# floe/backscrub

Hardware: AMD Instinct MI355X
Metric: composited frames/sec at 640×480 (batch), 1/2/4/8 MI355X + mask IoU vs CPU ref (higher is better)
Workload: dtype f32 (network) / u8 (image kernels)

## Files before the change

backscrub_amd/api.py:

```python
from __future__ import annotations

import ctypes as C
import os

import numpy as np

_HERE = os.path.dirname(os.path.abspath(__file__))
_LIB = None

_u8p = C.POINTER(C.c_uint8)
DEBUG_FN = C.CFUNCTYPE(None, C.c_void_p, C.c_char_p)
STAGE_FN = C.CFUNCTYPE(None, C.c_void_p)


class BsxError(RuntimeError):
    pass


class _Info(C.Structure):
    _fields_ = [("model_type", C.c_int), ("width", C.c_int), ("height", C.c_int), ("n_streams", C.c_int),
                ("in_w", C.c_int), ("in_h", C.c_int), ("in_c", C.c_int), ("out_w", C.c_int), ("out_h", C.c_int),
                ("out_c", C.c_int), ("roi", C.c_int * 4), ("in_roi", C.c_int * 4), ("n_ops", C.c_int), ("n_steps", C.c_int),
                ("device", C.c_int), ("norm_scale", C.c_float), ("norm_offset", C.c_float), ("nn_flops_per_frame", C.c_double),
                ("act_bytes_per_stream", C.c_size_t)]


class LaunchStat(C.Structure):
    _fields_ = [("name", C.c_char * 64), ("avg_ms", C.c_double), ("bytes", C.c_double), ("flops", C.c_double)]


SYMBOLS = [
    ("bsx_version", C.c_char_p, []),
    ("bsx_device_count", C.c_int, []),
    ("bsx_new", C.c_void_p, [C.c_char_p, C.c_size_t, C.c_size_t, C.c_size_t, C.c_int, C.c_int, DEBUG_FN, STAGE_FN, STAGE_FN, STAGE_FN, C.c_void_p]),
    ("bsx_delete", None, [C.c_void_p]),
    ("bsx_get_info", C.c_int, [C.c_void_p, C.POINTER(_Info)]),
    ("bsx_last_error", C.c_char_p, [C.c_void_p]),
    ("bsx_reset", C.c_int, [C.c_void_p, C.c_void_p]),
    ("bsx_process_host", C.c_int, [C.c_void_p, C.c_int, C.c_void_p, C.c_size_t, C.c_void_p, C.c_size_t]),
    ("bsx_process_batch", C.c_int, [C.c_void_p, C.c_void_p, C.c_int, C.c_void_p, C.c_void_p]),
    ("bsx_masks_device", C.c_void_p, [C.c_void_p]),
    ("bsx_composite_batch", C.c_int, [C.c_void_p, C.c_void_p, C.c_size_t, C.c_void_p, C.c_void_p, C.c_void_p, C.c_int, C.c_void_p]),
    ("bsx_step_batch", C.c_int, [C.c_void_p, C.c_void_p, C.c_void_p, C.c_size_t, C.c_void_p, C.c_int, C.c_void_p]),
    ("bsx_step_batch_yuyv", C.c_int, [C.c_void_p, C.c_void_p, C.c_void_p, C.c_size_t, C.c_void_p, C.c_int, C.c_void_p]),
    ("bsx_step_batch_ex", C.c_int, [C.c_void_p, C.c_void_p, C.c_void_p, C.c_size_t, C.c_void_p, C.c_int, C.c_void_p, C.c_uint]),
    ("bsx_step_batch_pipelined", C.c_int, [C.c_void_p, C.c_void_p, C.c_void_p, C.c_size_t, C.c_void_p, C.c_int, C.c_void_p, C.c_uint]),
    ("bsx_step_batch_vcam", C.c_int, [C.c_void_p, C.c_void_p, C.c_void_p, C.c_size_t, C.c_void_p, C.c_int, C.c_int, C.c_int, C.c_void_p, C.c_uint]),
    ("bsx_resize_bgr", C.c_int, [C.c_void_p, C.c_void_p, C.c_int, C.c_int, C.c_void_p, C.c_int, C.c_int, C.c_int, C.c_void_p]),
    ("bsx_bgr_to_yuyv", C.c_int, [C.c_void_p, C.c_void_p, C.c_void_p, C.c_int, C.c_int, C.c_int, C.c_void_p]),
    ("bsx_yuyv_to_bgr", C.c_int, [C.c_void_p, C.c_void_p, C.c_void_p, C.c_int, C.c_int, C.c_int, C.c_void_p]),
    ("bsx_background_load", C.c_void_p, [C.c_void_p, C.c_char_p, C.c_int]),
    ("bsx_background_from_frames", C.c_void_p, [C.c_void_p, C.c_void_p, C.c_int, C.c_int, C.c_int, C.c_double, C.c_int]),
    ("bsx_background_free", None, [C.c_void_p]),
    ("bsx_background_info", C.c_int, [C.c_void_p, C.POINTER(C.c_int), C.POINTER(C.c_int), C.POINTER(C.c_int), C.POINTER(C.c_double), C.POINTER(C.c_int)]),
    ("bsx_background_grab", C.c_int, [C.c_void_p, C.c_int, C.c_int, C.c_void_p, C.c_void_p]),
    ("bsx_media_decode", C.c_int, [C.c_char_p, C.POINTER(C.c_int), C.POINTER(C.c_int), C.POINTER(C.c_double), C.POINTER(C.POINTER(C.c_uint8)), C.c_char_p, C.c_size_t]),
    ("bsx_media_free", None, [C.POINTER(C.c_uint8)]),
    ("bsx_live_new", C.c_void_p, [C.c_void_p]),
    ("bsx_live_delete", None, [C.c_void_p]),
    ("bsx_live_set_input_frame", C.c_int, [C.c_void_p, C.c_void_p, C.c_size_t]),
    ("bsx_live_get_output_mask", C.c_int, [C.c_void_p, C.c_void_p, C.c_size_t]),
    ("bsx_live_timings", C.c_int, [C.c_void_p, C.POINTER(C.c_long), C.POINTER(C.c_long)]),
    ("bsx_gaussian_blur_bgr", C.c_int, [C.c_void_p, C.c_void_p, C.c_void_p, C.c_int, C.c_int, C.c_int, C.c_int, C.c_void_p]),
    ("bsx_debug_gauss_coeffs", C.c_int, [C.c_int, C.c_int, C.POINTER(C.c_uint32), C.POINTER(C.c_uint32)]),
    ("bsx_flip_bgr", C.c_int, [C.c_void_p, C.c_void_p, C.c_void_p, C.c_int, C.c_int, C.c_int, C.c_int, C.c_void_p]),
    ("bsx_debug_buffer", C.c_int, [C.c_void_p, C.c_int, C.POINTER(C.c_void_p), C.POINTER(C.c_size_t)]),
    ("bsx_debug_run_stage", C.c_int, [C.c_void_p, C.c_int, C.c_void_p, C.c_int, C.c_void_p]),
    ("bsx_plan_describe", C.c_char_p, [C.c_void_p]),
    ("bsx_debug_tensor", C.c_long, [C.c_void_p, C.c_int, C.POINTER(C.c_float), C.c_long]),
    ("bsx_model_precompile", C.c_int, [C.c_char_p, C.c_char_p, C.c_char_p, C.c_size_t]),
    ("bsx_model_kernel_source", C.c_long, [C.c_char_p, C.c_char_p, C.c_size_t]),
    ("bsx_model_seg_source", C.c_long, [C.c_char_p, C.c_char_p, C.c_size_t]),
    ("bsx_debug_tensor_of", C.c_long, [C.c_void_p, C.c_int, C.c_int, C.POINTER(C.c_float), C.c_long]),
    ("bsx_debug_mask_tile_stats", C.c_int, [C.c_void_p, C.c_int, C.POINTER(C.c_long)]),
    ("bsx_debug_program_timeline", C.c_int, [C.c_void_p, C.c_int, C.POINTER(C.c_ulonglong), C.c_int, C.c_void_p]),
    ("bsx_model_describe", C.c_int, [C.c_char_p, C.c_char_p, C.c_size_t]),
    ("bsx_profile_batch", C.c_int, [C.c_void_p, C.c_void_p, C.c_void_p, C.c_size_t, C.c_void_p, C.c_int, C.c_int, C.POINTER(LaunchStat), C.c_int, C.c_void_p]),
]


def lib_path() -> str:
    return os.environ.get("BSX_LIBRARY") or os.path.join(_HERE, "libbsx.so")


def lib():
    global _LIB
    if _LIB is None:
        import torch
        p = lib_path()
        if not os.path.exists(p):
            raise BsxError("libbsx.so is missing (%s): run `python -m backscrub_amd.build` — there is no CPU fallback" % p)
        L = C.CDLL(p)
        for name, res, args in SYMBOLS:
            f = getattr(L, name)
            f.restype = res
            f.argtypes = args
        _LIB = L
    return _LIB


def _check(rc, ctx=None, what=""):
    if rc != 0:
        msg = lib().bsx_last_error(ctx) or b""
        raise BsxError("%s failed (%d): %s" % (what, rc, msg.decode(errors="replace").strip()))


def _torch():
    import torch
    return torch


def _stream_ptr():
    torch = _torch()
    return C.c_void_p(torch.cuda.current_stream().cuda_stream)


class MaskGen:

    def __init__(self, model_path, width, height, n_streams=1, device=0, threads=2, ondebug=None, onprep=None, oninfer=None,
                 onmask=None, caller_ctx=None):
        L = lib()
        self._cbs = (DEBUG_FN(ondebug) if ondebug else DEBUG_FN(), STAGE_FN(onprep) if onprep else STAGE_FN(),
                     STAGE_FN(oninfer) if oninfer else STAGE_FN(), STAGE_FN(onmask) if onmask else STAGE_FN())
        self.h = L.bsx_new(os.fsencode(model_path), threads, width, height, n_streams, device, *self._cbs, caller_ctx)
        if not self.h:
            raise BsxError("bsx_new failed: %s" % (L.bsx_last_error(None) or b"").decode(errors="replace").strip())
        info = _Info()
        _check(L.bsx_get_info(self.h, C.byref(info)), self.h, "bsx_get_info")
        self.info = {k: (list(getattr(info, k)) if k in ("roi", "in_roi") else getattr(info, k)) for k, _ in _Info._fields_}
        self.width, self.height, self.n_streams, self.device = width, height, n_streams, device

    def process_batch(self, frames, masks_out=None):
        n = self._n(frames)
        mo = C.c_void_p(masks_out.data_ptr()) if masks_out is not None else None
        _check(lib().bsx_process_batch(self.h, C.c_void_p(frames.data_ptr()), n, mo, _stream_ptr()), self.h, "bsx_process_batch")
        return self.masks()[:n]

    def composite(self, bg, frames, masks=None, out=None):
        torch = _torch()
        n = self._n(frames)
        if out is None:
            out = torch.empty_like(frames)
        stride = self._bg(bg, n)
        mp = C.c_void_p(masks.data_ptr()) if masks is not None else None
        _check(lib().bsx_composite_batch(self.h, C.c_void_p(bg.data_ptr()), stride, C.c_void_p(frames.data_ptr()), mp,
                                         C.c_void_p(out.data_ptr()), n, _stream_ptr()), self.h, "bsx_composite_batch")
        return out

    def _bg(self, bg, n):
        ok = (bg.dtype == _torch().uint8 and bg.is_cuda and bg.dim() in (3, 4) and tuple(bg.shape[-3:]) == (self.height, self.width, 3)
              and tuple(bg.stride()[-3:]) == (self.width * 3, 3, 1) and (bg.dim() == 3 or bg.shape[0] >= n) and bg.device.index == self.device
              and (bg.dim() == 3 or bg.stride(0) >= 0))
        if not ok:
            raise BsxError("bg must be a cuda:%d uint8 tensor [%d,%d,3] or [>=%d,%d,%d,3] with contiguous images" % (self.device, self.height, self.width, n, self.height, self.width))
        return 0 if bg.dim() == 3 else int(bg.stride(0))

    def step(self, frames, bg, out):
# ... 95 lines not shown
        self._release_pending()

    def resize_bgr(self, src, dw, dh):
        torch = _torch()
        n, sh, sw, _ = src.shape
        dst = torch.empty((n, dh, dw, 3), dtype=torch.uint8, device=src.device)
        _check(lib().bsx_resize_bgr(self.h, C.c_void_p(src.data_ptr()), sw, sh, C.c_void_p(dst.data_ptr()), dw, dh, n, _stream_ptr()),
               self.h, "bsx_resize_bgr")
        return dst

    def bgr_to_yuyv(self, bgr):
        torch = _torch()
        n, h, w, _ = bgr.shape
        out = torch.empty((n, h, w, 2), dtype=torch.uint8, device=bgr.device)
        _check(lib().bsx_bgr_to_yuyv(self.h, C.c_void_p(bgr.data_ptr()), C.c_void_p(out.data_ptr()), w, h, n, _stream_ptr()),
               self.h, "bsx_bgr_to_yuyv")
        return out

    def flip_bgr(self, bgr, code):
        torch = _torch()
        n, h, w, _ = bgr.shape
        out = torch.empty_like(bgr)
        _check(lib().bsx_flip_bgr(self.h, C.c_void_p(bgr.data_ptr()), C.c_void_p(out.data_ptr()), w, h, n, int(code), _stream_ptr()), self.h, "bsx_flip_bgr")
        return out

    def gaussian_blur(self, bgr, ksize=25, out=None):
        torch = _torch()
        n, h, w, _ = bgr.shape
        if out is None:
            out = torch.empty_like(bgr)
        elif out.shape != bgr.shape or out.dtype != bgr.dtype or not out.is_contiguous() or out.device != bgr.device:
            raise BsxError("out must be a contiguous tensor shaped like the input")
        _check(lib().bsx_gaussian_blur_bgr(self.h, C.c_void_p(bgr.data_ptr()), C.c_void_p(out.data_ptr()), w, h, n, int(ksize), _stream_ptr()),
               self.h, "bsx_gaussian_blur_bgr")
        return out

    def yuyv_to_bgr(self, yuyv):
        torch = _torch()
        n, h, w, _ = yuyv.shape
        out = torch.empty((n, h, w, 3), dtype=torch.uint8, device=yuyv.device)
        _check(lib().bsx_yuyv_to_bgr(self.h, C.c_void_p(yuyv.data_ptr()), C.c_void_p(out.data_ptr()), w, h, n, _stream_ptr()),
               self.h, "bsx_yuyv_to_bgr")
        return out

    def process_host(self, frame: np.ndarray, stream_idx=0, mask_out: np.ndarray | None = None) -> np.ndarray:
        if frame.dtype != np.uint8 or frame.ndim != 3 or frame.shape[2] != 3 or frame.shape[0] != self.height or frame.shape[1] != self.width:
            raise BsxError("frame must be uint8 [%d,%d,3]" % (self.height, self.width))
        if frame.strides[2] != 1 or frame.strides[1] != 3:
            frame = np.ascontiguousarray(frame)
        if mask_out is None:
            mask_out = np.empty((self.height, self.width), np.uint8)
        elif (not isinstance(mask_out, np.ndarray) or mask_out.dtype != np.uint8 or mask_out.shape != (self.height, self.width)
              or mask_out.strides[1] != 1 or mask_out.strides[0] < self.width or not mask_out.flags.writeable):
            raise BsxError("mask_out must be a writable uint8 [%d,%d] array with unit inner stride" % (self.height, self.width))
        _check(lib().bsx_process_host(self.h, stream_idx, frame.ctypes.data, frame.strides[0], mask_out.ctypes.data, mask_out.strides[0]),
               self.h, "bsx_process_host")
        return mask_out

    def run_stage(self, stage, frames=None, n=None):
        n = n if n is not None else (self._n(frames, yuyv_in=(stage == 4)) if frames is not None else self.n_streams)
        fp = C.c_void_p(frames.data_ptr()) if frames is not None else None
        _check(lib().bsx_debug_run_stage(self.h, stage, fp, n, _stream_ptr()), self.h, "bsx_debug_run_stage")

    def input_tensor(self):
        i = self.info
        return self._view(0, "float32", (self.n_streams, i["in_h"], i["in_w"], i["in_c"]))

    def output_tensor(self):
        i = self.info
        return self._view(1, "float32", (self.n_streams, i["out_h"], i["out_w"], i["out_c"]))

    def ofinal(self):
        i = self.info
        return self._view(2, "uint8", (self.n_streams, i["out_h"], i["out_w"]))

    def plan(self) -> str:
        return lib().bsx_plan_describe(self.h).decode()

    def mask_tile_stats(self, n=None) -> dict:
        a = (C.c_long * 4)()
        _check(lib().bsx_debug_mask_tile_stats(self.h, n or self.n_streams, a), self.h, "bsx_debug_mask_tile_stats")
        return {"tiles": a[0], "uniform_255": a[1], "uniform_0": a[2], "general": a[3], "tile": "128x32"}

    def graph_tensor(self, idx, stream=None) -> np.ndarray:
        if stream is not None:
            n = lib().bsx_debug_tensor_of(self.h, idx, stream, None, 0)
            if n < 0:
                raise BsxError("tensor %d not materialised" % idx)
            a = np.empty(n, np.float32)
            lib().bsx_debug_tensor_of(self.h, idx, stream, a.ctypes.data_as(C.POINTER(C.c_float)), n)
            return a
        n = lib().bsx_debug_tensor(self.h, idx, None, 0)
        if n < 0:
            raise BsxError("tensor %d not materialised" % idx)
        _torch().cuda.synchronize()
        a = np.empty(n, np.float32)
        lib().bsx_debug_tensor(self.h, idx, a.ctypes.data_as(C.POINTER(C.c_float)), n)
        return a

    def _view(self, which, dtype, shape):
        torch = _torch()
        p, b = C.c_void_p(), C.c_size_t()
        _check(lib().bsx_debug_buffer(self.h, which, C.byref(p), C.byref(b)), self.h, "bsx_debug_buffer")
        return _as_torch(p.value, b.value, dtype, shape, self.device)

    def _n(self, frames, yuyv_in=False):
        ch = 2 if yuyv_in else 3
        if frames.dim() != 4 or tuple(frames.shape[1:]) != (self.height, self.width, ch) or not frames.is_contiguous() or not frames.is_cuda or frames.dtype != _torch().uint8:
            raise BsxError("frames must be a contiguous cuda uint8 tensor [n,%d,%d,%d]" % (self.height, self.width, ch))
        if frames.shape[0] > self.n_streams:
            raise BsxError("batch larger than n_streams")
        return int(frames.shape[0])

    def close(self):
        if getattr(self, "h", None):
            lib().bsx_delete(self.h)
            self.h = None

    def __del__(self):
        try:
            self.close()
        except Exception:
            pass


class _CudaArray:

    def __init__(self, ptr, nbytes, typestr, shape):
        self.__cuda_array_interface__ = {"shape": tuple(shape), "typestr": typestr, "data": (ptr, False), "version": 2, "strides": None}
        self._nbytes = nbytes


def _as_torch(ptr, nbytes, dtype, shape, device):
    torch = _torch()
    typestr = {"uint8": "|u1", "float32": "<f4"}[dtype]
    return torch.as_tensor(_CudaArray(ptr, nbytes, typestr, shape), device="cuda:%d" % device)


def media_decode(path: str):
    w, h, fps, ptr = C.c_int(), C.c_int(), C.c_double(), C.POINTER(C.c_uint8)()
    err = C.create_string_buffer(512)
    n = lib().bsx_media_decode(os.fsencode(path), C.byref(w), C.byref(h), C.byref(fps), C.byref(ptr), err, len(err))
    if n <= 0:
        raise BsxError(err.value.decode(errors="replace") or "media decode failed (%d)" % n)
    try:
        frames = np.ctypeslib.as_array(ptr, (n, h.value, w.value, 3)).copy()
    finally:
        lib().bsx_media_free(ptr)
    return frames, fps.value


class Background:

    def __init__(self, mg: MaskGen, path=None, frames=None, fps=0.0, debug=0):
        self.mg = mg
        if path is not None:
            self.h = lib().bsx_background_load(mg.h, os.fsencode(path), debug)
        else:
            frames = np.ascontiguousarray(frames, np.uint8)
            n, hh, ww, _ = frames.shape
            self.h = lib().bsx_background_from_frames(mg.h, frames.ctypes.data, ww, hh, n, float(fps), debug)
        if not self.h:
            raise BsxError("cannot load background")
        w, h, n, f, v = C.c_int(), C.c_int(), C.c_int(), C.c_double(), C.c_int()
        lib().bsx_background_info(self.h, C.byref(w), C.byref(h), C.byref(n), C.byref(f), C.byref(v))
        self.width, self.height, self.n_frames, self.fps, self.video = w.value, h.value, n.value, f.value, bool(v.value)
# ... 130 lines not shown
```

backscrub_amd/csrc/bsx_api.hip:

```cpp
#include "debug_switches.hpp"
#include <hip/hip_runtime.h>

#include <cmath>
#include <cstdarg>
#include <cstdio>
#include <cstdlib>
#include <cstring>
#include <map>
#include <memory>
#include <string>
#include <vector>

#include "../../include/bsx.h"
#include "gen_mid.hpp"
#include "gen_seg.hpp"
#include "kernels.hpp"
#include "roctx_ranges.hpp"
#include "rtc.hpp"
#include "plan.hpp"
#include "tflite_model.hpp"

using namespace bsx;

namespace {
thread_local std::string g_last_error;

struct HostResizeTab {
  std::vector<int> xofs, yofs;
  std::vector<short> xa, ya;
  int sw = 0, sh = 0, dw = 0, dh = 0, mode = 0;
};

inline int cv_floor(float v) { int i = (int)v; return i - (i > v); }
inline short sat_short(long v) { return (short)(v < -32768 ? -32768 : (v > 32767 ? 32767 : v)); }

HostResizeTab make_resize_tab(int sw, int sh, int dw, int dh) {
  HostResizeTab t;
  t.sw = sw; t.sh = sh; t.dw = dw; t.dh = dh;
  if (sw == dw && sh == dh) { t.mode = 1; return t; }
  double inv_x = (double)dw / sw, inv_y = (double)dh / sh;
  double scale_x = 1. / inv_x, scale_y = 1. / inv_y;
  long isx = lrint(scale_x), isy = lrint(scale_y);
  bool area_fast = std::fabs(scale_x - (double)isx) < 2.220446049250313e-16 && std::fabs(scale_y - (double)isy) < 2.220446049250313e-16;
  if (area_fast && isx == 2 && isy == 2) { t.mode = 2; return t; }
  t.xofs.resize(dw); t.xa.resize(2 * (size_t)dw); t.yofs.resize(dh); t.ya.resize(2 * (size_t)dh);
  for (int dx = 0; dx < dw; dx++) {
    float fx = (float)((dx + 0.5) * scale_x - 0.5);
    int sx = cv_floor(fx);
    fx -= sx;
    if (sx < 0) { fx = 0; sx = 0; }
    if (sx >= sw - 1) { fx = 0; sx = sw - 1; }
    t.xofs[dx] = sx;
    t.xa[2 * dx] = sat_short(lrintf((1.f - fx) * 2048.f));
    t.xa[2 * dx + 1] = sat_short(lrintf(fx * 2048.f));
  }
  for (int dy = 0; dy < dh; dy++) {
    float fy = (float)((dy + 0.5) * scale_y - 0.5);
    int sy = cv_floor(fy);
    fy -= sy;
    t.yofs[dy] = sy;
    t.ya[2 * dy] = sat_short(lrintf((1.f - fy) * 2048.f));
    t.ya[2 * dy + 1] = sat_short(lrintf(fy * 2048.f));
  }
  return t;
}

struct DevResizeTab {
  ResizeTab tab;
  void* mem = nullptr;
};
struct VcamTab {
  DevResizeTab d;
  bool direct = false;
};

}

struct bsx_ctx {
  bsx_debug_fn ondebug = nullptr;
  bsx_stage_fn onprep = nullptr, oninfer = nullptr, onmask = nullptr;
  void* caller_ctx = nullptr;
  Graph graph;
  Plan plan;
  int model_type = BSX_MODEL_UNKNOWN;
  float norm_scale = 0, norm_offset = 0;
  int width = 0, height = 0, n_streams = 0, device = 0;
  int inW = 0, inH = 0, inC = 0, outW = 0, outH = 0, outC = 0;
  Rect4 roi{}, in_roi{};
  size_t threads = 0;
  hipStream_t own_stream = nullptr;
// ... 63 lines not shown
  DeviceGuard& operator=(const DeviceGuard&) = delete;
};

void report(bsx_ctx* c, bsx_debug_fn fn, void* user, const char* fmt, ...) {
  char buf[1024];
  va_list ap;
  va_start(ap, fmt);
  vsnprintf(buf, sizeof buf, fmt, ap);
  va_end(ap);
  if (c) c->last_error = buf;
  g_last_error = buf;
  if (fn) fn(user, buf); else fputs(buf, stderr);
}

#define BSX_HIP(c, expr)                                                                                    \
  do {                                                                                                      \
    hipError_t e_ = (expr);                                                                                 \
    if (e_ != hipSuccess) {                                                                                 \
      report((c), (c) ? (c)->ondebug : nullptr, (c) ? (c)->caller_ctx : nullptr, "error: HIP %s at %s:%d (%s)\n", \
             hipGetErrorString(e_), __FILE__, __LINE__, #expr);                                             \
      return BSX_EDEVICE;                                                                                   \
    }                                                                                                       \
  } while (0)

int upload_tab(bsx_ctx* c, const HostResizeTab& h, DevResizeTab* d) {
  d->tab.sw = h.sw; d->tab.sh = h.sh; d->tab.dw = h.dw; d->tab.dh = h.dh; d->tab.mode = h.mode;
  if (h.mode != 0) return BSX_OK;
  d->tab.tile_ok = (mask_tile_fits(h.xofs.data(), h.yofs.data(), h.sw, h.sh, h.dw, h.dh) && !c->no_mask_tile) ? 1 : 0;
  d->tab.tile_class = nullptr;
  size_t b_xofs = h.xofs.size() * 4, b_yofs = h.yofs.size() * 4, b_xa = h.xa.size() * 2, b_ya = h.ya.size() * 2;
  auto up16 = [](size_t v) { return (v + 15) / 16 * 16; };
  size_t total = up16(b_xofs) + up16(b_yofs) + up16(b_xa) + up16(b_ya);
  BSX_HIP(c, hipMalloc(&d->mem, total));
  char* p = (char*)d->mem;
  BSX_HIP(c, hipMemcpy(p, h.xofs.data(), b_xofs, hipMemcpyHostToDevice)); d->tab.xofs = (const int*)p; p += up16(b_xofs);
  BSX_HIP(c, hipMemcpy(p, h.yofs.data(), b_yofs, hipMemcpyHostToDevice)); d->tab.yofs = (const int*)p; p += up16(b_yofs);
  BSX_HIP(c, hipMemcpy(p, h.xa.data(), b_xa, hipMemcpyHostToDevice)); d->tab.xa = (const short*)p; p += up16(b_xa);
  BSX_HIP(c, hipMemcpy(p, h.ya.data(), b_ya, hipMemcpyHostToDevice)); d->tab.ya = (const short*)p;
  return BSX_OK;
}

std::string build_seg_kernels(const Plan& plan, bool h16, bool u8in, const std::string& arch, std::vector<char>* code, bool* cached, size_t* src_bytes = nullptr) {
  std::string why, log;
  if (BSX_DBG_ENV("BSX_NO_SEG_RTC")) return "ahead-of-time kernels (BSX_NO_SEG_RTC)";
  const std::string src = generate_seg_source(plan, h16, u8in, &why);
  if (src.empty()) return "ahead-of-time kernels (" + why + ")";
  if (src_bytes) *src_bytes = src.size();
  if (!rtc_build(src, arch, code, &log, cached)) { if (BSX_DBG_ENV("BSX_RTC_DEBUG")) fprintf(stderr, "%s\n", log.c_str()); return "ahead-of-time kernels (hipRTC: " + log.substr(0, 600) + ")"; }
  return "";
}

struct MidBuild { std::vector<char> code; std::string source, note; bool cached = false, opaque_tid = false; long scratch = -1; };
std::string build_mid_kernel(const Plan& plan, bool act16, const std::string& arch, MidBuild* out) {
  std::string why, log;
  int force = -1;
  if (const char* e = BSX_DBG_ENV("BSX_RTC_TID")) force = atoi(e) != 0;
  auto build = [&](bool opaque, MidBuild* b) -> std::string {
    b->source = generate_mid_source(plan, &why, act16, opaque);
    if (b->source.empty()) return "interpreted (" + why + ")";
    if (!rtc_build(b->source, arch, &b->code, &log, &b->cached)) { if (BSX_DBG_ENV("BSX_RTC_DEBUG")) fprintf(stderr, "%s\n", log.c_str()); return "interpreted (hipRTC: " + log.substr(0, 400) + ")"; }
    b->opaque_tid = opaque;
    b->scratch = code_object_scratch_bytes(b->code, "bsx_mid");
    return "";
  };
  std::string err = build(force == 1, out);
  if (!err.empty() || force >= 0 || out->scratch <= 0) return err;
  MidBuild alt;
  if (build(true, &alt).empty() && alt.scratch >= 0 && alt.scratch < out->scratch) *out = std::move(alt);
  return "";
}

int model_type_from_name(const std::string& n) {
  if (n.find("body-pix") != n.npos) return BSX_MODEL_BODYPIX;
  if (n.find("deeplab") != n.npos) return BSX_MODEL_DEEPLAB;
  if (n.find("segm_") != n.npos) return BSX_MODEL_MEET;
  if (n.find("selfie") != n.npos) return BSX_MODEL_MLKIT;
  return BSX_MODEL_UNKNOWN;
}

int init_device_state(bsx_ctx* c) {
  BSX_HIP(c, hipStreamCreateWithFlags(&c->own_stream, hipStreamNonBlocking));
  const size_t N = (size_t)c->n_streams;
  BSX_HIP(c, hipMalloc(&c->d_arena, c->plan.arena_floats_per_stream * N * sizeof(float)));
  BSX_HIP(c, hipMalloc(&c->d_net_in, N * c->inW * c->inH * c->inC * sizeof(float)));
  BSX_HIP(c, hipMalloc(&c->d_net_in_u8, N * c->inW * c->inH * sizeof(uint32_t)));
  BSX_HIP(c, hipMalloc(&c->d_net_out, N * c->outW * c->outH * c->outC * sizeof(float)));
  BSX_HIP(c, hipMalloc(&c->d_weights, std::max<size_t>(c->plan.weights.size(), 4) * sizeof(float)));
  BSX_HIP(c, hipMemcpy(c->d_weights, c->plan.weights.data(), c->plan.weights.size() * sizeof(float), hipMemcpyHostToDevice));
  BSX_HIP(c, hipMalloc(&c->d_weights16, std::max<size_t>(c->plan.weights16.size(), 8) * sizeof(uint16_t)));
  BSX_HIP(c, hipMemcpy(c->d_weights16, c->plan.weights16.data(), c->plan.weights16.size() * sizeof(uint16_t), hipMemcpyHostToDevice));
  if (const char* m = getenv("BSX_F16_GEMM")) c->f16_terms = !strcmp(m, "off") ? 0 : (!strcmp(m, "fast") ? 1 : (!strcmp(m, "fast16") ? 17 : 3));
  c->use_program = !c->plan.program.empty() && BSX_DBG_ENV("BSX_NO_FRAME_PROGRAM") == nullptr &&
                   (c->plan.seg.on || c->plan.program_lds_tensors >= c->plan.program_global_tensors || BSX_DBG_ENV("BSX_FORCE_FRAME_PROGRAM") != nullptr);
  if (c->use_program) {
    BSX_HIP(c, hipMalloc(&c->d_program, c->plan.program.size() * sizeof(MicroOp)));
    BSX_HIP(c, hipMemcpy(c->d_program, c->plan.program.data(), c->plan.program.size() * sizeof(MicroOp), hipMemcpyHostToDevice));
    BSX_HIP(c, frame_program_prepare(c->plan.program_lds_floats));
    if (c->plan.seg.on) BSX_HIP(c, seg_prepare());
    const char* a16 = getenv("BSX_ACT16");
    c->act16 = a16 && atoi(a16) != 0 && c->plan.seg.on;
    if (!BSX_DBG_ENV("BSX_NO_RTC")) {
      hipDeviceProp_t prop;
      MidBuild mb;
      if (hipGetDeviceProperties(&prop, c->device) != hipSuccess) c->mid_note = "interpreted (no device properties)";
      else {
        const std::string err = build_mid_kernel(c->plan, c->act16, prop.gcnArchName, &mb);
        if (!err.empty()) c->mid_note = err;
        else if (rtc_load(mb.code, "bsx_mid", &c->mid) != hipSuccess) { c->mid_note = "interpreted (code object did not load)"; (void)hipGetLastError(); }
        else c->mid_note = std::string("specialised kernel (hipRTC") + (mb.cached ? ", from the cache" : ", compiled now") + (mb.opaque_tid ? ", lane indices re-derived per op" : "") +
                           (mb.scratch > 0 ? ", " + std::to_string(mb.scratch) + " B of scratch" : "") + ")";
      }
    } else c->mid_note = "interpreted (BSX_NO_RTC)";
    if (c->act16 && !c->mid.fn) {
      c->last_error = "BSX_ACT16: the specialised middle kernel is not available (" + c->mid_note + ")";
      return BSX_EDEVICE;
    }
    if (c->act16) c->mid_note += ", 16-bit activation storage";
  } else {
    BSX_HIP(c, nn_prepare());
  }
  if (const char* l = BSX_DBG_ENV("BSX_PIPE_WGS")) c->pipe_wgs = std::min(8, std::max(0, atoi(l)));
  if (const char* l = BSX_DBG_ENV("BSX_LANES")) c->lanes = std::min(4, std::max(1, atoi(l)));
  if (c->lanes > 1) {
    BSX_HIP(c, hipEventCreateWithFlags(&c->ev_fork, hipEventDisableTiming));
    for (int k = 1; k < c->lanes; k++) {
      BSX_HIP(c, hipStreamCreateWithFlags(&c->lane_stream[k], hipStreamNonBlocking));
      BSX_HIP(c, hipEventCreateWithFlags(&c->ev_join[k], hipEventDisableTiming));
    }
  }
  if (BSX_DBG_ENV("BSX_NO_GRAPH")) c->graph_state = -1;
  c->in_u8 = BSX_DBG_ENV("BSX_F32_INPUT") == nullptr && ((c->use_program && c->plan.seg.on) || (!c->use_program && head0_u8_ok(c->plan)));
  if (c->use_program && c->plan.seg.on) {
    if (BSX_DBG_ENV("BSX_NO_RTC")) c->seg_note = "ahead-of-time kernels (BSX_NO_RTC)";
    else {
      hipDeviceProp_t prop;
      std::vector<char> code;
      bool cached = false;
      if (hipGetDeviceProperties(&prop, c->device) != hipSuccess) c->seg_note = "ahead-of-time kernels (no device properties)";
      else {
        c->seg_note = build_seg_kernels(c->plan, c->act16, c->in_u8, prop.gcnArchName, &code, &cached);
        if (c->seg_note.empty()) {
          if (rtc_load(code, "bsx_seg_head", &c->seg_mod) != hipSuccess || rtc_function(c->seg_mod, "bsx_seg_k2", &c->seg_fn[0]) != hipSuccess ||
              rtc_function(c->seg_mod, "bsx_seg_k3", &c->seg_fn[1]) != hipSuccess || rtc_function(c->seg_mod, "bsx_seg_tail", &c->seg_fn[2]) != hipSuccess) {
            rtc_unload(&c->seg_mod);
            (void)hipGetLastError();
            c->seg_note = "ahead-of-time kernels (code object did not load)";
          } else c->seg_note = std::string("specialised kernels (hipRTC") + (cached ? ", from the cache)" : ", compiled now)");
        }
      }
    }
  }
  BSX_HIP(c, hipMalloc(&c->d_ofinal, N * c->outW * c->outH));
  BSX_HIP(c, hipMalloc(&c->d_masks, N * c->width * c->height));
  BSX_HIP(c, hipMemset(c->d_ofinal, 0, N * c->outW * c->outH));
  BSX_HIP(c, hipMemset(c->d_masks, 255, N * c->width * c->height));
  {
    const double sigma_color = 100.0, sigma_space = 100.0;
    const double gc = -0.5 / (sigma_color * sigma_color), gs = -0.5 / (sigma_space * sigma_space);
    const int radius = 2;
    std::vector<float> lut(768);
    for (int i = 0; i < 768; i++) lut[i] = (float)std::exp(i * i * gc);
    BSX_HIP(c, hipMalloc(&c->d_color_lut, 768 * sizeof(float)));
    BSX_HIP(c, hipMemcpy(c->d_color_lut, lut.data(), 768 * sizeof(float), hipMemcpyHostToDevice));
    int k = 0;
    for (int i = -radius; i <= radius; i++) for (int j = -radius; j <= radius; j++) {
      double r = std::sqrt((double)i * i + (double)j * j);
// ... 9 lines not shown
  int rc = upload_tab(c, make_resize_tab(c->roi.w, c->roi.h, c->in_roi.w, c->in_roi.h), &c->tab_down);
  if (rc) return rc;
  rc = upload_tab(c, make_resize_tab(c->in_roi.w, c->in_roi.h, c->roi.w, c->roi.h), &c->tab_up);
  if (rc) return rc;
  c->tiles_per_frame = (size_t)((c->roi.w + mask_tile_width() - 1) / mask_tile_width()) * (size_t)((c->roi.h + mask_tile_height() - 1) / mask_tile_height());
  if (!c->no_uniform_tiles && c->tab_up.tab.mode == 0 && c->tab_up.tab.tile_ok) {
    BSX_HIP(c, hipMalloc(&c->d_tile_class, N * c->tiles_per_frame + 4));
    BSX_HIP(c, hipMemset(c->d_tile_class, 0, N * c->tiles_per_frame + 4));
    c->tab_up.tab.tile_class = c->d_tile_class;
  }
  return BSX_OK;
}

hipStream_t pick(bsx_ctx*, void* s) { return (hipStream_t)s; }

int run_prep(bsx_ctx* c, const uint8_t* d_frames, int n, hipStream_t s, bool with_f32 = false, bool yuyv_in = false) {
  bsx_roctx::Range range("bsx:prep");
  float* f32 = (!c->in_u8 || with_f32) ? c->tensor_ptr(c->plan.input) : nullptr;
  uint32_t* u8 = c->in_u8 ? c->d_net_in_u8 : nullptr;
  BSX_HIP(c, launch_prep_fused(d_frames, c->width, c->height, c->roi, f32, u8, c->inW, c->inH, c->in_roi, c->tab_down.tab, c->bilateral, n, s, yuyv_in));
  return BSX_OK;
}
bool argmax_tail(const bsx_ctx* c) {
  return !c->use_program && !c->keep_logits && c->model_type == BSX_MODEL_DEEPLAB && !c->plan.steps.empty() && c->plan.steps.back().out == c->plan.output &&
         resize_argmax_fusable(c->plan.steps.back());
}
hipError_t launch_program(bsx_ctx* c, int n, hipStream_t s, unsigned long long* timeline = nullptr) {
  long pf = (long)c->plan.arena_floats_per_stream;
  if (c->mid.fn) {
    float* arena = c->d_arena;
    const float* weights = c->d_weights;
    void* args[] = {&arena, &pf, &weights, &timeline};
    return hipModuleLaunchKernel(c->mid.fn, (unsigned)n, 1, 1, (unsigned)c->plan.mid_lanes, 1, 1, 0, s, args, nullptr);
  }
  return launch_frame_program(c->d_program, (int)c->plan.program.size(), c->plan.program_lds_floats, c->d_arena, pf, c->d_net_in, c->d_net_out, c->d_weights, n, s,
                              timeline);
}
int state_write_fence(bsx_ctx* c, hipStream_t s) {
  if (!c->wait_before_state) return BSX_OK;
  hipEvent_t ev = c->wait_before_state;
  c->wait_before_state = nullptr;
  BSX_HIP(c, hipStreamWaitEvent(s, ev, 0));
  return BSX_OK;
}
bool infer_decodes(const bsx_ctx* c) { return (c->use_program && c->plan.seg.on && !c->keep_logits) || argmax_tail(c); }
hipError_t seg_launch(hipFunction_t fn, int tiles, int n, int lds_floats, hipStream_t s, void** args) {
  return hipModuleLaunchKernel(fn, (unsigned)tiles * (unsigned)n, 1, 1, kSegThreads, 1, 1, (unsigned)((size_t)lds_floats * sizeof(float)), s, args, nullptr);
}
hipError_t seg_head(bsx_ctx* c, int n, hipStream_t s) {
  const SegPlan& sp = c->plan.seg;
  long pf = (long)c->plan.arena_floats_per_stream;
  if (!c->seg_mod.fn)
    return launch_seg_head(sp.head, c->d_arena, pf, c->in_u8 ? (const void*)c->d_net_in_u8 : (const void*)c->d_net_in, c->d_weights, n, s, c->act16, c->in_u8, c->norm_scale, c->norm_offset);
  SegHead d = sp.head; float* arena = c->d_arena; const float* in = c->in_u8 ? reinterpret_cast<const float*>(c->d_net_in_u8) : c->d_net_in; const float* w = c->d_weights;
  float sc = c->norm_scale, of = c->norm_offset; int nf = n;
  void* args[] = {&d, &arena, &pf, &in, &w, &sc, &of, &nf};
  return seg_launch(c->seg_mod.fn, d.tiles_y * d.tiles_x, n, d.lds_floats, s, args);
}
hipError_t seg_k2(bsx_ctx* c, int n, hipStream_t s) {
  const SegPlan& sp = c->plan.seg;
  long pf = (long)c->plan.arena_floats_per_stream;
  if (!c->seg_fn[0]) return launch_seg_k2(sp.k2, c->d_arena, pf, c->d_weights, n, s, c->act16);
  SegK2 d = sp.k2; float* arena = c->d_arena; const float* w = c->d_weights; int nf = n;
  void* args[] = {&d, &arena, &pf, &w, &nf};
  return seg_launch(c->seg_fn[0], d.tiles_y * d.tiles_x, n, d.lds_floats, s, args);
}
hipError_t seg_k3(bsx_ctx* c, int n, hipStream_t s) {
  const SegPlan& sp = c->plan.seg;
  long pf = (long)c->plan.arena_floats_per_stream;
  if (!c->seg_fn[1]) return launch_seg_k3(sp.k3, c->d_arena, pf, c->d_weights, n, s, c->act16);
  SegK3 d = sp.k3; float* arena = c->d_arena; const float* w = c->d_weights; int nf = n;
  void* args[] = {&d, &arena, &pf, &w, &nf};
  return seg_launch(c->seg_fn[1], d.tiles_y * d.tiles_x, n, d.lds_floats, s, args);
}
hipError_t seg_tail(bsx_ctx* c, uint8_t* ofinal, bool logits, int n, hipStream_t s) {
  const SegPlan& sp = c->plan.seg;
  long pf = (long)c->plan.arena_floats_per_stream;
  if (logits || !c->seg_fn[2]) return launch_seg_tail(sp.tail, c->d_arena, pf, c->d_net_out, ofinal, c->d_weights, logits, n, s, c->act16);
  SegTail d = sp.tail; float* arena = c->d_arena; float* no = c->d_net_out; const float* w = c->d_weights; int nf = n;
  void* args[] = {&d, &arena, &pf, &no, &ofinal, &w, &nf};
  return seg_launch(c->seg_fn[2], d.tiles_y * d.tiles_x, n, d.lds_floats, s, args);
}

int run_infer(bsx_ctx* c, int n, hipStream_t s, bool logits = true, int slot = 0) {
  bsx_roctx::Range range("bsx:network");
  if (c->use_program && c->plan.seg.on) {
    const SegPlan& sp = c->plan.seg;
    const long pf = (long)c->plan.arena_floats_per_stream;
    BSX_HIP(c, seg_head(c, n, s));
    BSX_HIP(c, seg_k2(c, n, s));
    BSX_HIP(c, launch_program(c, n, s));
    BSX_HIP(c, seg_k3(c, n, s));
    if (sp.tail.pre_gate_off >= 0) BSX_HIP(c, launch_seg_gate(sp.tail.gate, c->d_arena, pf, c->d_weights, sp.tail.pre_gate_off, n, s));
    if (!logits) { const int frc = state_write_fence(c, s); if (frc) return frc; }
    BSX_HIP(c, seg_tail(c, c->d_ofinal + (size_t)slot * c->outW * c->outH, logits, n, s));
    return BSX_OK;
  }
  if (c->use_program) {
    BSX_HIP(c, launch_program(c, n, s));
    return BSX_OK;
  }
  const bool fused_tail = !logits && argmax_tail(c);
  const size_t ns = c->plan.steps.size() - (fused_tail ? 1 : 0);
  for (size_t i = 0; i < ns; i++)
    BSX_HIP(c, launch_step(c->plan.steps[i], c->plan, c->d_arena, c->d_net_in, c->d_net_out, c->d_weights, n, c->n_streams, s, c->d_weights16, c->f16_terms, c->in_u8 ? c->d_net_in_u8 : nullptr, c->norm_scale, c->norm_offset));
  if (fused_tail) {
    const Step& last = c->plan.steps.back();
    { const int frc = state_write_fence(c, s); if (frc) return frc; }
    BSX_HIP(c, launch_resize_argmax_iir(last, c->d_arena + (size_t)c->plan.tensor_off[last.in0] * (size_t)c->n_streams,
                                        c->d_ofinal + (size_t)slot * c->outW * c->outH, n, s, c->tail_generic));
  }
  return BSX_OK;
}
int run_decode(bsx_ctx* c, int n, hipStream_t s, int slot = 0) {
  bsx_roctx::Range range("bsx:decode");
  { const int frc = state_write_fence(c, s); if (frc) return frc; }
  BSX_HIP(c, launch_decode(c->model_type, c->tensor_ptr(c->plan.output), c->d_ofinal + (size_t)slot * c->outW * c->outH, c->outW * c->outH, c->outC, n, s));
  return BSX_OK;
}
ResizeTab tab_up_at(const bsx_ctx* c, int slot) {
  ResizeTab t = c->tab_up.tab;
  if (t.tile_class) t.tile_class += (size_t)slot * c->tiles_per_frame;
  return t;
}
int run_mask(bsx_ctx* c, int n, hipStream_t s, int slot = 0) {
  bsx_roctx::Range range("bsx:mask");
  BSX_HIP(c, launch_mask_upscale_blur(c->d_ofinal + (size_t)slot * c->outW * c->outH, c->outW, c->outH, c->in_roi, tab_up_at(c, slot),
                                      c->d_masks + (size_t)slot * c->width * c->height, c->width, c->height, c->roi, n, s));
  return BSX_OK;
}
int process_impl(bsx_ctx* c, const uint8_t* d_frames, int n, int slot, hipStream_t s, bool yuyv_in = false) {
  int rc;
  if ((rc = run_prep(c, d_frames, n, s, false, yuyv_in))) return rc;
  if (c->onprep) { BSX_HIP(c, hipStreamSynchronize(s)); c->onprep(c->caller_ctx); }
  const bool fused_decode = infer_decodes(c);
  if ((rc = run_infer(c, n, s, !fused_decode, slot))) return rc;
  if (c->oninfer) { BSX_HIP(c, hipStreamSynchronize(s)); c->oninfer(c->caller_ctx); }
  if (!fused_decode && (rc = run_decode(c, n, s, slot))) return rc;
  if (c->onmask) { BSX_HIP(c, hipStreamSynchronize(s)); c->onmask(c->caller_ctx); }
  return run_mask(c, n, s, slot);
}

}

namespace {
std::string mid_barrier_line(const Plan& p, bool act16) {
  std::string why;
  const std::string src = generate_mid_source(p, &why, act16);
  if (src.empty()) return "specialised middle kernel: none (" + why + ")\n";
  const size_t k0 = src.find("extern \"C\" __global__");
  auto count = [&](const char* pat) { size_t n = 0; for (size_t q = src.find(pat, k0); q != std::string::npos; q = src.find(pat, q + 1)) n++; return n; };
  const size_t ob = count("op_barrier();"), sy = count("__syncthreads();");
  char line[256];
  snprintf(line, sizeof line, "specialised middle kernel: %zu micro-ops, %zu workgroup barriers per launch (%zu between ops + %zu inside ops)\n", p.program.size(), ob + sy, ob, sy);
  return line;
}
}

extern "C" {

const char* bsx_version(void) { return "bsx 0.1 (HIP gfx950, f32 NHWC)"; }

int bsx_device_count(void) {
  int n = 0;
  if (hipGetDeviceCount(&n) != hipSuccess) return 0;
  return n;
}

const char* bsx_last_error(const bsx_ctx* ctx) { return ctx ? ctx->last_error.c_str() : g_last_error.c_str(); }

bsx_ctx* bsx_new(const char* model_path, size_t threads, size_t width, size_t height, int n_streams, int device, bsx_debug_fn ondebug,
                 bsx_stage_fn onprep, bsx_stage_fn oninfer, bsx_stage_fn onmask, void* caller_ctx) {
  if (!model_path || !width || !height || n_streams <= 0 || n_streams > 65535) {
    report(nullptr, ondebug, caller_ctx, "error: bad arguments to bsx_new\n"); return nullptr; }
  try {
  std::unique_ptr<bsx_ctx> c(new bsx_ctx);
// ... 442 lines not shown

int bsx_resize_bgr(bsx_ctx* c, const uint8_t* d_src, int sw, int sh, uint8_t* d_dst, int dw, int dh, int n, void* stream) {
  if (!c || !d_src || !d_dst || sw <= 0 || sh <= 0 || dw <= 0 || dh <= 0 || n <= 0) return BSX_EINVAL;
  DeviceGuard guard(c->device);
  auto key = std::make_pair(std::make_pair(sw, sh), std::make_pair(dw, dh));
  auto it = c->bg_tabs.find(key);
  if (it == c->bg_tabs.end()) {
    DevResizeTab d;
    int rc = upload_tab(c, make_resize_tab(sw, sh, dw, dh), &d);
    if (rc) return rc;
    it = c->bg_tabs.emplace(key, d).first;
  }
  BSX_HIP(c, launch_resize_bgr(d_src, d_dst, it->second.tab, n, pick(c, stream)));
  return BSX_OK;
}

int bsx_flip_bgr(bsx_ctx* c, const uint8_t* d_src, uint8_t* d_dst, int w, int h, int n, int code, void* stream) {
  if (!c || !d_src || !d_dst || d_src == d_dst || w <= 0 || h <= 0 || n <= 0) return BSX_EINVAL;
  DeviceGuard guard(c->device);
  BSX_HIP(c, launch_flip_bgr(d_src, d_dst, w, h, code, n, pick(c, stream)));
  return BSX_OK;
}

int bsx_gaussian_blur_bgr(bsx_ctx* c, const uint8_t* d_src, uint8_t* d_dst, int w, int h, int n, int ksize, void* stream) {
  if (!c || !d_src || !d_dst || d_src == d_dst || w <= 0 || h <= 0 || n <= 0 || ksize < 1 || ksize > 31 || !(ksize & 1)) return BSX_EINVAL;
  DeviceGuard guard(c->device);
  BSX_HIP(c, launch_gauss_blur(d_src, d_dst, w, h, ksize, n, pick(c, stream)));
  return BSX_OK;
}

int bsx_bgr_to_yuyv(bsx_ctx* c, const uint8_t* d_bgr, uint8_t* d_yuyv, int w, int h, int n, void* stream) {
  if (!c || !d_bgr || !d_yuyv || w <= 0 || h <= 0 || n <= 0) return BSX_EINVAL;
  DeviceGuard guard(c->device);
  BSX_HIP(c, launch_bgr_to_yuyv(d_bgr, d_yuyv, w, h, n, pick(c, stream)));
  return BSX_OK;
}

int bsx_yuyv_to_bgr(bsx_ctx* c, const uint8_t* d_yuyv, uint8_t* d_bgr, int w, int h, int n, void* stream) {
  if (!c || !d_yuyv || !d_bgr || w <= 0 || h <= 0 || n <= 0 || (((long)w * h) & 1)) return BSX_EINVAL;
  DeviceGuard guard(c->device);
  BSX_HIP(c, launch_yuyv_to_bgr(d_yuyv, d_bgr, w, h, n, pick(c, stream)));
  return BSX_OK;
}

int bsx_debug_buffer(bsx_ctx* c, int which, void** d_ptr, size_t* bytes) {
  if (!c || !d_ptr || !bytes) return BSX_EINVAL;
  const size_t N = (size_t)c->n_streams;
  switch (which) {
    case 0: *d_ptr = c->tensor_ptr(c->plan.input); *bytes = N * c->inW * c->inH * c->inC * 4; break;
    case 1: *d_ptr = c->tensor_ptr(c->plan.output); *bytes = N * c->outW * c->outH * c->outC * 4; break;
    case 2: *d_ptr = c->d_ofinal; *bytes = N * c->outW * c->outH; break;
    case 3: *d_ptr = c->d_masks; *bytes = N * c->width * c->height; break;
    default: return BSX_EINVAL;
  }
  return BSX_OK;
}

int bsx_debug_run_stage(bsx_ctx* c, int stage, const uint8_t* d_frames, int n, void* stream) {
  if (!c || n <= 0 || n > c->n_streams) return BSX_EINVAL;
  if (stage >= 1 && stage <= 3 && c->pend.active) { c->last_error = "error: a pipelined composite is pending (flush with bsx_step_batch_pipelined(ctx, NULL, ...) first)\n"; return BSX_EINVAL; }
  DeviceGuard guard(c->device);
  hipStream_t s = pick(c, stream);
  switch (stage) {
    case 0: if (!d_frames) return BSX_EINVAL; return run_prep(c, d_frames, n, s, true);
    case 1: return run_infer(c, n, s);
    case 2: return run_decode(c, n, s);
    case 3: return run_mask(c, n, s);
    case 4:
      if (!d_frames || !prep_yuyv_fusable(c->width, c->roi, c->tab_down.tab)) return BSX_EINVAL;
      return run_prep(c, d_frames, n, s, true, true);
    default: return BSX_EINVAL;
  }
}

int bsx_profile_batch(bsx_ctx* c, const uint8_t* d_frames, const uint8_t* d_bg, size_t bg_stride, uint8_t* d_out, int n, int iters,
                      bsx_launch_stat* out, int cap, void* stream) {
  if (!c || !d_frames || !d_bg || !d_out || !out || n <= 0 || n > c->n_streams || iters <= 0) return BSX_EINVAL;
  if (c->pend.active) { c->last_error = "error: a pipelined composite is pending (flush with bsx_step_batch_pipelined(ctx, NULL, ...) first)\n"; return BSX_EINVAL; }
  DeviceGuard guard(c->device);
  hipStream_t s = pick(c, stream);
  const bool seg = c->use_program && c->plan.seg.on;
  const bool fused_decode = infer_decodes(c);
  const bool atail = argmax_tail(c);
  const int n_net = c->use_program ? (seg ? (c->plan.seg.tail.pre_gate_off >= 0 ? 6 : 5) : 1) : (int)c->plan.steps.size();
  const bool fuse_tail = !c->onmask && !c->no_mask_blend_fusion &&
                         mask_blend_fusable(c->width, c->height, c->roi, d_bg, bg_stride, d_frames, d_out);
  const int L = 1 + n_net + (fused_decode ? 0 : 1) + (fuse_tail ? 1 : 2) + (fuse_tail ? 1 : 0);
  if (cap < L) return BSX_EINVAL;
  std::vector<hipEvent_t> ev((size_t)L + 1);
  for (auto& e : ev) BSX_HIP(c, hipEventCreate(&e));
  std::vector<double> sum(L, 0.0);
  const double N = n, px = (double)c->width * c->height;
  for (int it = 0; it < iters; it++) {
    int k = 0;
    BSX_HIP(c, hipEventRecord(ev[0], s));
#define BSX_TIMED(call)                                    \
    do {                                                   \
      BSX_HIP(c, (call));                                  \
      BSX_HIP(c, hipEventRecord(ev[k + 1], s));            \
      k++;                                                 \
    } while (0)
    BSX_TIMED(launch_prep_fused(d_frames, c->width, c->height, c->roi, c->in_u8 ? nullptr : c->tensor_ptr(c->plan.input), c->in_u8 ? c->d_net_in_u8 : nullptr, c->inW, c->inH, c->in_roi,
                                c->tab_down.tab, c->bilateral, n, s));
    const long pf = (long)c->plan.arena_floats_per_stream;
    if (seg) {
      const SegPlan& sp = c->plan.seg;
      BSX_TIMED(seg_head(c, n, s));
      BSX_TIMED(seg_k2(c, n, s));
      BSX_TIMED(launch_program(c, n, s));
      BSX_TIMED(seg_k3(c, n, s));
      if (sp.tail.pre_gate_off >= 0) BSX_TIMED(launch_seg_gate(sp.tail.gate, c->d_arena, pf, c->d_weights, sp.tail.pre_gate_off, n, s));
      BSX_TIMED(seg_tail(c, c->d_ofinal, !fused_decode, n, s));
    } else if (c->use_program)
      BSX_TIMED(launch_program(c, n, s));
    else {
      for (size_t si = 0; si + (atail ? 1 : 0) < c->plan.steps.size(); si++)
        BSX_TIMED(launch_step(c->plan.steps[si], c->plan, c->d_arena, c->d_net_in, c->d_net_out, c->d_weights, n, c->n_streams, s, c->d_weights16, c->f16_terms, c->in_u8 ? c->d_net_in_u8 : nullptr, c->norm_scale, c->norm_offset));
      if (atail) BSX_TIMED(launch_resize_argmax_iir(c->plan.steps.back(), c->d_arena + (size_t)c->plan.tensor_off[c->plan.steps.back().in0] * (size_t)c->n_streams,
                                                    c->d_ofinal, n, s, c->tail_generic));
    }
    if (!fused_decode) BSX_TIMED(launch_decode(c->model_type, c->tensor_ptr(c->plan.output), c->d_ofinal, c->outW * c->outH, c->outC, n, s));
    if (fuse_tail) {
      BSX_TIMED(launch_mask_blend(c->d_ofinal, c->outW, c->outH, c->in_roi, c->tab_up.tab, c->d_masks, c->width, c->height, c->roi, d_bg, bg_stride,
                                  d_frames, d_out, n, s));
      BSX_TIMED(launch_blend(d_bg, bg_stride, d_frames, c->d_masks, d_out, (size_t)c->width * c->height, n, s));
    } else {
      BSX_TIMED(launch_mask_upscale_blur(c->d_ofinal, c->outW, c->outH, c->in_roi, c->tab_up.tab, c->d_masks, c->width, c->height, c->roi, n, s));
      BSX_TIMED(launch_blend(d_bg, bg_stride, d_frames, c->d_masks, d_out, (size_t)c->width * c->height, n, s));
    }
#undef BSX_TIMED
    BSX_HIP(c, hipStreamSynchronize(s));
    for (int j = 0; j < L; j++) { float ms = 0; BSX_HIP(c, hipEventElapsedTime(&ms, ev[j], ev[j + 1])); sum[j] += ms; }
  }
  for (auto& e : ev) (void)hipEventDestroy(e);
  auto put = [&](int j, const std::string& name, double bytes, double flops) {
    memset(&out[j], 0, sizeof out[j]);
    snprintf(out[j].name, sizeof out[j].name, "%s", name.c_str());
    out[j].avg_ms = sum[j] / iters; out[j].bytes = bytes; out[j].flops = flops;
  };
  int j = 0;
  const double canvas = (double)c->inW * c->inH;
  const double touched = (double)std::min(c->roi.w, 2 * c->in_roi.w) * (double)std::min(c->roi.h, 2 * c->in_roi.h);
  put(j++, "prep", N * (3.0 * touched + (c->in_u8 ? 4.0 : 12.0) * canvas), 0);
  if (seg) {
    const std::vector<Step>& S = c->plan.steps;
    const int NS = (int)S.size();
    auto macs = [&](int a, int b) { double m = 0; for (int i = a; i <= b; i++) m += S[i].macs; return m; };
    const SegPlan& sp = c->plan.seg;
    const double eA = 16.0 * sp.head.H1 * sp.head.W1, eb0 = 16.0 * sp.head.H2 * sp.head.W2, ec0 = (double)sp.k2.dw.C * sp.k2.H3 * sp.k2.W3;
    const double elo2 = 16.0 * sp.k3.HL * sp.k3.WL, elo = 16.0 * sp.k3.H2 * sp.k3.W2;
    const double ein = (double)c->inW * c->inH * c->inC, eout = (double)c->outW * c->outH * c->outC;
    put(j++, "seg_head", N * ((c->in_u8 ? 4.0 * c->inW * c->inH : 4.0 * ein) + 4.0 * (eA + eb0)), N * 2.0 * macs(0, 2));
    put(j++, "seg_k2", N * 4.0 * (eb0 + eb0 + ec0), N * 2.0 * macs(3, 8));
    put(j++, "frame_program", N * 4.0 * (ec0 + elo2) + 4.0 * c->plan.weights.size(), N * 2.0 * macs(9, NS - 11));
    put(j++, "seg_k3", N * 4.0 * (eb0 + elo2 + elo), N * 2.0 * macs(NS - 10, NS - 8));
    if (sp.tail.pre_gate_off >= 0) put(j++, "seg_gate", N * 4.0 * (16.0 * (sp.tail.gate.part[0].n + sp.tail.gate.part[1].n) + 16.0), 0);
    put(j++, fused_decode ? "seg_tail+decode" : "seg_tail", N * (4.0 * (eA + elo) + (fused_decode ? 2.0 * c->outW * c->outH : 4.0 * eout)), N * 2.0 * macs(NS - 7, NS - 1));
  } else if (c->use_program) {
    double io = (double)c->inW * c->inH * c->inC + (double)c->outW * c->outH * c->outC;
    put(j++, "frame_program", N * io * 4.0 + 4.0 * c->plan.weights.size(), N * 2.0 * c->plan.macs_per_frame);
  } else
  for (const Step& st : c->plan.steps) {
    double in = (double)st.H * st.W * st.Cin, o = (double)st.OH * st.OW * st.Cout, b = 0;
    switch (st.kind) {
      case StepKind::Eltwise: b = in + o + (st.elt == kEltUnary ? 0 : (st.bcast1 ? st.Cin : in)) + (st.elt == kEltMulAdd ? in : 0); break;
      case StepKind::Concat: b = 2 * o; break;
      case StepKind::Gap: b = in + st.Cin; break;
      default: b = in + o + (st.residual >= 0 ? o : 0) + (st.in_scale >= 0 ? st.Cin : 0); break;
    }
    const bool is_tail = atail && &st == &c->plan.steps.back();
    const bool ir_on = c->d_weights16 && c->f16_terms > 0;
    const bool h0 = c->plan.steps[0].fuse_head0;
    const bool h0_member = h0 && (&st == &c->plan.steps[1] || &st == &c->plan.steps[2]);
    if (h0_member || (st.fused_away && !(h0 && &st <= &c->plan.steps[2]) && ir_on)) { put(j++, st.label + " (inside the launch before)", 0, 0); continue; }
    if (st.chain_mid >= 0 && chain3_on(c->plan, st.chain_mid, n, c->d_weights16, c->f16_terms)) { put(j++, st.label + " (inside the chained launch)", 0, 0); continue; }
    if (st.chain_first >= 0 && chain3_on(c->plan, (int)(&st - c->plan.steps.data()), n, c->d_weights16, c->f16_terms)) {
      const Step& ca = c->plan.steps[st.chain_first];
      const Step& cc = c->plan.steps[st.chain_last];
      put(j++, ca.label + "+" + st.label + "+" + cc.label, N * 4.0 * ((double)ca.H * ca.W * ca.Cin + (double)cc.OH * cc.OW * cc.Cout), N * 2.0 * (ca.macs + st.macs + cc.macs));
      continue;
    }
    if (st.fuse_head0 && h0) {
      const Step& d1 = c->plan.steps[1];
      const Step& p2 = c->plan.steps[2];
      put(j++, st.label + "+" + d1.label + "+" + p2.label, N * ((c->in_u8 ? 4.0 * st.H * st.W : 4.0 * in) + 4.0 * (double)p2.OH * p2.OW * p2.Cout), N * 2.0 * (st.macs + d1.macs + p2.macs));
      continue;
    }
    if (st.fuse_dw >= 0 && ir_on) {
      const Step& dd = c->plan.steps[st.fuse_dw];
      put(j++, st.label + "+" + dd.label, N * 4.0 * (in + (double)dd.OH * dd.OW * dd.Cout), N * 2.0 * (st.macs + dd.macs));
      continue;
    }
    put(j++, is_tail ? st.label + "+argmax" : st.label, is_tail ? N * (4.0 * in + 2.0 * st.OH * st.OW) : N * b * 4.0, N * 2.0 * st.macs);
  }
  if (!fused_decode) put(j++, "decode_iir", N * ((double)c->outW * c->outH * c->outC * 4.0 + 2.0 * c->outW * c->outH), 0);
  if (fuse_tail) {
    put(j++, "mask_blend", N * ((double)c->in_roi.w * c->in_roi.h + 10.0 * px), 0);
    put(j++, "blend(standalone)", N * 10.0 * px, 0);
  } else {
    put(j++, "mask_upscale_blur", N * ((double)c->in_roi.w * c->in_roi.h + (double)c->roi.w * c->roi.h), 0);
    put(j++, "blend", N * 10.0 * px, 0);
  }
  return j;
}

int bsx_debug_mask_tile_stats(bsx_ctx* c, int n, long* out4) {
  if (!c || !out4 || n <= 0 || n > c->n_streams) return BSX_EINVAL;
  DeviceGuard guard(c->device);
  out4[0] = (long)c->tiles_per_frame * n; out4[1] = out4[2] = 0; out4[3] = out4[0];
  if (!c->d_tile_class) return BSX_OK;
  BSX_HIP(c, launch_tile_class(c->d_ofinal, c->outW, c->outH, c->in_roi, c->tab_up.tab, c->roi, n, nullptr));
  std::vector<uint8_t> cls((size_t)out4[0]);
  if (hipDeviceSynchronize() != hipSuccess || hipMemcpy(cls.data(), c->d_tile_class, cls.size(), hipMemcpyDeviceToHost) != hipSuccess) return BSX_EDEVICE;
  out4[3] = 0;
  for (uint8_t v : cls) out4[v == 1 ? 1 : (v == 2 ? 2 : 3)]++;
  return BSX_OK;
}

int bsx_debug_gauss_coeffs(int ksize, int shift, uint32_t* c4, uint32_t* c2) {
  return (c4 && c2 && gauss_coeff_words(ksize, shift, c4, c2)) ? BSX_OK : BSX_EINVAL;
}

int bsx_debug_program_timeline(bsx_ctx* c, int n, unsigned long long* ticks, int cap, void* stream) {
  if (!c || !ticks || n <= 0 || n > c->n_streams) return BSX_EINVAL;
  DeviceGuard guard(c->device);
  if (!c->use_program) return 0;
  const int L = (int)c->plan.program.size();
  if (cap < L + 1 || L + 1 > 256) return BSX_EINVAL;
  unsigned long long* d = nullptr;
  const size_t kTl = 1024 + 64 * 16 * 4;
  BSX_HIP(c, hipMalloc(&d, kTl * sizeof(unsigned long long)));
  BSX_HIP(c, hipMemset(d, 0, kTl * sizeof(unsigned long long)));
  hipStream_t s = pick(c, stream);
  BSX_HIP(c, launch_program(c, n, s, d));
  BSX_HIP(c, hipStreamSynchronize(s));
  BSX_HIP(c, hipMemcpy(ticks, d, std::min((size_t)cap, kTl) * sizeof(unsigned long long), hipMemcpyDeviceToHost));
  (void)hipFree(d);
  return L;
}

int bsx_model_describe(const char* model_path, char* buf, size_t cap) {
  if (!model_path || !buf || !cap) return BSX_EINVAL;
  std::string err, out;
  int rc = BSX_OK;
  try {
  Graph g; Plan p;
  if (!load_tflite(model_path, &g, &err) || !build_plan(g, &p, &err)) { out = err; rc = BSX_EMODEL; }
  else {
    char head[256];
    snprintf(head, sizeof head, "ops=%d nodes=%d steps=%d macs=%.0f arena_floats=%zu\n", g.n_file_ops, (int)g.nodes.size(), (int)p.steps.size(),
             p.macs_per_frame, p.arena_floats_per_stream);
    out = head + p.describe();
    snprintf(head, sizeof head, "program micro-ops=%zu lds_floats=%d lds_tensors=%d hbm_tensors=%d arena_bytes_per_frame=%ld placement_policy=%u lds_blocks=%zu lds_check=%s\n", p.program.size(),
             p.program_lds_floats, p.program_lds_tensors, p.program_global_tensors, p.program_arena_bytes, p.program_policy, p.program_blocks.size(), p.program_check.c_str());
    out += head;
    for (size_t i = 0; i < p.program_labels.size(); i++) out += "P" + std::to_string(i) + " " + p.program_labels[i] + "\n";
    if (p.seg.on) out += p.seg_text;
    if (!p.program.empty()) out += mid_barrier_line(p, false);
    if (BSX_DBG_ENV("BSX_PLAN_BLOCKS"))
      for (const auto& b : p.program_blocks) { snprintf(head, sizeof head, "block off=%d len=%d steps=[%d,%d] %s\n", b.off, b.len, b.from, b.until, b.what.c_str()); out += head; }
  }
  } catch (const std::exception& e) { out = std::string("exception while reading the model: ") + e.what(); rc = BSX_EMODEL; }
  catch (...) { out = "unknown exception while reading the model"; rc = BSX_EMODEL; }
  snprintf(buf, cap, "%s", out.c_str());
  return rc;
}

long bsx_model_kernel_source(const char* model_path, char* buf, size_t cap) {
  if (!model_path || !buf || !cap) return BSX_EINVAL;
  try {
    Graph g; Plan p;
    std::string err, why;
    if (!load_tflite(model_path, &g, &err) || !build_plan(g, &p, &err)) { snprintf(buf, cap, "%s", err.c_str()); return BSX_EMODEL; }
    const char* a16 = getenv("BSX_ACT16");
    if (p.program.empty()) { snprintf(buf, cap, "no program"); return 0; }
    MidBuild mb;
    const std::string e = build_mid_kernel(p, a16 && atoi(a16) != 0 && p.seg.on, "gfx950", &mb);
    if (!e.empty()) {
      const std::string src = generate_mid_source(p, &why, a16 && atoi(a16) != 0 && p.seg.on);
      if (src.empty()) { snprintf(buf, cap, "%s", why.c_str()); return 0; }
      snprintf(buf, cap, "%s", src.c_str());
      return (long)src.size();
    }
    snprintf(buf, cap, "%s", mb.source.c_str());
    return (long)mb.source.size();
  } catch (...) { snprintf(buf, cap, "exception while reading the model"); return BSX_EMODEL; }
}

long bsx_model_seg_source(const char* model_path, char* buf, size_t cap) {
  if (!model_path || !buf || !cap) return BSX_EINVAL;
  try {
    Graph g; Plan p;
    std::string err, why;
    if (!load_tflite(model_path, &g, &err) || !build_plan(g, &p, &err)) { snprintf(buf, cap, "%s", err.c_str()); return BSX_EMODEL; }
    const char* a16 = getenv("BSX_ACT16");
    const std::string src = generate_seg_source(p, a16 && atoi(a16) != 0 && p.seg.on, BSX_DBG_ENV("BSX_F32_INPUT") == nullptr, &why);
    if (src.empty()) { snprintf(buf, cap, "%s", why.c_str()); return 0; }
    snprintf(buf, cap, "%s", src.c_str());
// ... 67 lines not shown
```

backscrub_amd/csrc/gen_seg.cpp:

```cpp
#include "gen_seg.hpp"

#include <cstdarg>
#include <cstdio>

namespace bsx {
namespace {

const char kSegSource[] =
#include "seg_rtc_src.inc"
    ;

}

std::string seg_constants_text(const SegPlan& sp, const char* pre) {
  std::string out;
  auto P = [&](const char* fmt, ...) {
    char buf[1024];
    va_list ap;
    va_start(ap, fmt);
    vsnprintf(buf, sizeof buf, fmt, ap);
    va_end(ap);
    out += buf;
  };
  auto conv = [&](const char* n, const SegConvW& c) { P("  t.%s.w_off = %lldll; t.%s.b_off = %lldll; t.%s.Cin = %d; t.%s.Cout = %d; t.%s.cout_pad = %d; t.%s.act = %d;\n", n, c.w_off, n, c.b_off, n, c.Cin, n, c.Cout, n, c.cout_pad, n, c.act); };
  auto dw = [&](const char* n, const SegDwW& c) { P("  t.%s.w_off = %lldll; t.%s.b_off = %lldll; t.%s.C = %d; t.%s.act = %d;\n", n, c.w_off, n, c.b_off, n, c.C, n, c.act); };
  auto gate = [&](const char* n, const SegGate& g_) {
    P("  t.%s.n_parts = %d; t.%s.sum_parts = %d; t.%s.n_fc = %d; t.%s.timing_skip = 0;\n", n, g_.n_parts, n, g_.sum_parts, n, g_.n_fc, n);
    for (int i = 0; i < 2; i++) {
      P("  t.%s.part[%d].off = %lldll; t.%s.part[%d].n = %d; t.%s.part[%d].C = %d; t.%s.part[%d].hw = (float)%.9g;\n", n, i, g_.part[i].off, n, i, g_.part[i].n, n, i, g_.part[i].C, n, i, (double)g_.part[i].hw);
      P("  t.%s.fc[%d].w_off = %lldll; t.%s.fc[%d].b_off = %lldll; t.%s.fc[%d].Cin = %d; t.%s.fc[%d].Cout = %d; t.%s.fc[%d].act = %d;\n", n, i, g_.fc[i].w_off, n, i, g_.fc[i].b_off, n, i, g_.fc[i].Cin, n, i,
              g_.fc[i].Cout, n, i, g_.fc[i].act);
    }
  };
  const SegHead& H = sp.head; const SegK2& K2 = sp.k2; const SegK3& K3 = sp.k3; const SegTail& T = sp.tail;
  P("// segment descriptors of the loaded graph as constants (gen_seg.cpp: seg_constants_text)\nconstexpr SegHead %sHEAD = [] { SegHead t{};\n", pre);
  P("  t.H0 = %d; t.W0 = %d; t.H1 = %d; t.W1 = %d; t.H2 = %d; t.W2 = %d; t.stem_pt = %d; t.stem_pl = %d; t.dw_pt = %d; t.dw_pl = %d;\n", H.H0, H.W0, H.H1, H.W1, H.H2, H.W2, H.stem_pt, H.stem_pl, H.dw_pt, H.dw_pl);
  conv("stem", H.stem); conv("pw", H.pw); dw("dw", H.dw);
  P("  t.a_off = %lldll; t.b0_off = %lldll; t.part_a_off = %lldll; t.part_b0_off = %lldll; t.TR = %d; t.TC = %d; t.tiles_y = %d; t.tiles_x = %d; t.lds_floats = %d; t.rw = %d; t.m_ct = %uu;\n  return t; }();\n",
          H.a_off, H.b0_off, H.part_a_off, H.part_b0_off, H.TR, H.TC, H.tiles_y, H.tiles_x, H.lds_floats, H.rw, H.m_ct);
  P("constexpr SegK2 %sK2 = [] { SegK2 t{};\n  t.H2 = %d; t.W2 = %d; t.H3 = %d; t.W3 = %d; t.dw_pt = %d; t.dw_pl = %d;\n", pre, K2.H2, K2.W2, K2.H3, K2.W3, K2.dw_pt, K2.dw_pl);
  gate("gate", K2.gate); conv("pw_a", K2.pw_a); conv("pw_b", K2.pw_b); dw("dw", K2.dw);
  P("  t.b0_off = %lldll; t.B_off = %lldll; t.c0_off = %lldll; t.part_B_off = %lldll; t.TR = %d; t.TC = %d; t.tiles_y = %d; t.tiles_x = %d; t.lds_floats = %d; t.rw = %d; t.m_ct = %uu;\n  return t; }();\n",
          K2.b0_off, K2.B_off, K2.c0_off, K2.part_B_off, K2.TR, K2.TC, K2.tiles_y, K2.tiles_x, K2.lds_floats, K2.rw, K2.m_ct);
  P("constexpr SegK3 %sK3 = [] { SegK3 t{};\n  t.H2 = %d; t.W2 = %d; t.HL = %d; t.WL = %d; t.half_pixel = %d; t.align_corners = %d;\n", pre, K3.H2, K3.W2, K3.HL, K3.WL, K3.half_pixel, K3.align_corners);
  conv("pw1", K3.pw1); conv("pw2", K3.pw2); dw("dw", K3.dw);
  P("  t.skip_off = %lldll; t.lo2_off = %lldll; t.g_off = %lldll; t.lo_off = %lldll; t.part_lo_off = %lldll; t.TR = %d; t.TC = %d; t.tiles_y = %d; t.tiles_x = %d; t.lds_floats = %d; t.lo_floats = %d; t.hs = (float)%.9g; t.ws = (float)%.9g;\n  return t; }();\n",
          K3.skip_off, K3.lo2_off, K3.g_off, K3.lo_off, K3.part_lo_off, K3.TR, K3.TC, K3.tiles_y, K3.tiles_x, K3.lds_floats, K3.lo_floats, (double)K3.hs, (double)K3.ws);
  P("constexpr SegTail %sTAIL = [] { SegTail t{};\n  t.H1 = %d; t.W1 = %d; t.HL = %d; t.WL = %d; t.H0 = %d; t.W0 = %d; t.half_pixel = %d; t.align_corners = %d;\n", pre, T.H1, T.W1, T.HL, T.WL, T.H0, T.W0, T.half_pixel, T.align_corners);
  gate("gate", T.gate); conv("pw", T.pw); dw("dw", T.dw);
  P("  t.tc_w_off = %lldll; t.tc_b_off = %lldll; t.Co = %d; t.act3 = %d; t.model_type = %d; t.skip_off = %lldll; t.lo_off = %lldll; t.pre_gate_off = %lldll; t.TR = %d; t.TC = %d; t.tiles_y = %d; t.tiles_x = %d; "
             "t.lds_floats = %d; t.lo_floats = %d; t.hs = (float)%.9g; t.ws = (float)%.9g;\n  return t; }();\n",
          T.tc_w_off, T.tc_b_off, T.Co, T.act3, T.model_type, T.skip_off, T.lo_off, T.pre_gate_off, T.TR, T.TC, T.tiles_y, T.tiles_x, T.lds_floats, T.lo_floats, (double)T.hs, (double)T.ws);
  return out;
}

std::string generate_seg_source(const Plan& plan, bool h16, bool u8in, std::string* why) {
  auto fail = [&](const char* m) { if (why) *why = m; return std::string(); };
  if (!plan.seg.on) return fail("no segment kernels in this plan");
  const SegPlan& sp = plan.seg;
  const bool sig = sp.tail.act3 == kActSigmoid;
  if (!((sp.tail.Co == 2 && !sig) || sp.tail.Co == 1)) return fail("transpose-convolution output channels");
  std::string src = kSegSource;
  const std::string mark = "BSXS_SEG_CONSTANTS";
  const size_t at = src.find(mark);
  if (at == std::string::npos) return fail("embedded source has no constants marker");
  src.replace(at, mark.size(), seg_constants_text(sp, "kSeg"));
  char head[512];
  snprintf(head, sizeof head, "#define BSXS_SEG_RTC 1\n#define BSXS_SEG_HS %d\n#define BSXS_SEG_H16 %d\n#define BSXS_SEG_U8 %d\n#define BSXS_SEG_SIG %d\n#define BSXS_SEG_CO %d\n",
           sp.head.stem.act == kActHswish ? 1 : 0, h16 ? 1 : 0, u8in ? 1 : 0, sig ? 1 : 0, sp.tail.Co);
  return std::string(head) + src;
}

}
```

backscrub_amd/csrc/kernels.hpp:

```cpp
#pragma once
#include <hip/hip_runtime.h>

#include <cstddef>
#include <cstdint>

#include "plan.hpp"
#include "segments.hpp"

namespace bsx {

hipError_t launch_step(const Step& st, const Plan& plan, float* arena, float* net_in, float* net_out, const float* weights, int n, int n_cap,
                       hipStream_t s, const uint16_t* weights16 = nullptr, int f16_terms = 0, const uint32_t* net_in_u8 = nullptr, float in_scale = 0.f, float in_offset = 0.f);
inline bool head0_u8_ok(const Plan& plan) {
  if (plan.steps.empty() || !plan.steps[0].fuse_head0) return false;
  const Step& st = plan.steps[0];
  return st.in0 == plan.input && (long)(2 * (head0_band_rows(st.W, st.OW) + 2) + 1) * st.W <= 4 * 3 * 512;
}

inline bool chain3_on(const Plan& plan, int mid, int n, const uint16_t* weights16, int f16_terms) {
  if (mid < 0 || mid >= (int)plan.steps.size() || plan.steps[mid].chain_first < 0) return false;
  const Step& b = plan.steps[mid];
  const long M = (long)n * b.OH * b.OW;
  return weights16 && (f16_terms & 15) == 3 && M >= 8192 && M * plan.steps[b.chain_first].Cin < (1l << 31);
}

bool resize_argmax_fusable(const Step& st);
hipError_t launch_resize_argmax_iir(const Step& st, const float* lowres_logits, uint8_t* ofinal, int n, hipStream_t s, bool generic = false);

hipError_t frame_program_prepare(int lds_floats);
hipError_t launch_frame_program(const MicroOp* d_ops, int n_ops, int lds_floats, float* arena, long per_frame_floats, float* net_in, float* net_out,
                                const float* weights, int n, hipStream_t s, unsigned long long* timeline = nullptr);

hipError_t seg_prepare();
hipError_t nn_prepare();
hipError_t launch_seg_head(const SegHead& d, float* arena, long per_frame, const void* net_in, const float* weights, int n, hipStream_t s, bool h16 = false, bool u8 = false,
                           float in_scale = 0.f, float in_offset = 0.f);
hipError_t launch_seg_k2(const SegK2& d, float* arena, long per_frame, const float* weights, int n, hipStream_t s, bool h16 = false);
hipError_t launch_seg_k3(const SegK3& d, float* arena, long per_frame, const float* weights, int n, hipStream_t s, bool h16 = false);
hipError_t launch_seg_gate(const SegGate& gt, float* arena, long per_frame, const float* weights, long long out_off, int n, hipStream_t s);
hipError_t launch_seg_tail(const SegTail& d, float* arena, long per_frame, float* net_out, uint8_t* ofinal, const float* weights, bool logits, int n, hipStream_t s, bool h16 = false);

struct ResizeTab {
  const int* xofs = nullptr;
  const short* xa = nullptr;
  const int* yofs = nullptr;
  const short* ya = nullptr;
  int sw = 0, sh = 0, dw = 0, dh = 0;
  int mode = 0;
  int tile_ok = 0;
  uint8_t* tile_class = nullptr;
};
bool mask_tile_fits(const int* xofs, const int* yofs, int sw, int sh, int dw, int dh);
int mask_tile_width();
int mask_tile_height();
struct Rect4;
hipError_t launch_tile_class(const uint8_t* ofinal, int outW, int outH, const Rect4& in_roi, const ResizeTab& tab, const Rect4& roi, int n, hipStream_t s);

struct Rect4 { int x, y, w, h; };

struct BilateralParams {
  float space_w[13];
  int off_y[13], off_x[13];
  const float* color_lut;
  float scale, offset;
};

constexpr int kCanvasPad = 2;
bool bilateral_taps_match(const BilateralParams& bp);
hipError_t launch_prep_fused(const uint8_t* frames, int W, int H, Rect4 roi, float* input, uint32_t* input_u8, int inW, int inH, Rect4 in_roi, ResizeTab tab,
                             BilateralParams bp, int n, hipStream_t s, bool yuyv_in = false);
bool prep_yuyv_fusable(int W, Rect4 roi, const ResizeTab& tab);
hipError_t launch_decode(int model_type, const float* logits, uint8_t* ofinal, int npix, int nch, int n, hipStream_t s);
hipError_t launch_mask_upscale_blur(const uint8_t* ofinal, int outW, int outH, Rect4 in_roi, ResizeTab tab, uint8_t* mask, int W, int H,
                                    Rect4 roi, int n, hipStream_t s);
bool mask_blend_fusable(int W, int H, Rect4 roi, const uint8_t* bg, size_t bg_stride, const uint8_t* frames, const uint8_t* out);
hipError_t launch_mask_blend(const uint8_t* ofinal, int outW, int outH, Rect4 in_roi, ResizeTab tab, uint8_t* mask, int W, int H, Rect4 roi,
                             const uint8_t* bg, size_t bg_stride, const uint8_t* frames, uint8_t* out, int n, hipStream_t s, int yuyv = 0, int lds_pad = 0);
hipError_t launch_blend(const uint8_t* bg, size_t bg_stride, const uint8_t* frames, const uint8_t* masks, uint8_t* out, size_t npix,
                        int n, hipStream_t s);
hipError_t launch_resize_bgr(const uint8_t* src, uint8_t* dst, ResizeTab tab, int n, hipStream_t s);
hipError_t launch_bgr_to_yuyv(const uint8_t* bgr, uint8_t* yuyv, int w, int h, int n, hipStream_t s);
hipError_t launch_yuyv_to_bgr(const uint8_t* yuyv, uint8_t* bgr, int w, int h, int n, hipStream_t s);
hipError_t launch_flip_bgr(const uint8_t* src, uint8_t* dst, int w, int h, int code, int n, hipStream_t s);
hipError_t launch_gauss_blur(const uint8_t* src, uint8_t* dst, int w, int h, int ksize, int n, hipStream_t s);
bool gauss_coeff_words(int ksize, int shift, uint32_t* c4 , uint32_t* c2 );
bool gauss_blend_fusable(const uint8_t* frames, const uint8_t* masks, const uint8_t* out, int w, int ksize);
hipError_t launch_gauss_blend(const uint8_t* frames, const uint8_t* masks, uint8_t* out, int w, int h, int ksize, int n, hipStream_t s);
bool vcam_tile_fits(const int* xofs, const int* yofs, int sw, int sh, int dw, int dh);
hipError_t launch_vcam_blend_resize(const uint8_t* frames, bool yuyv_in, const uint8_t* bg, size_t bg_stride, const uint8_t* masks, uint8_t* out, int W, int H,
                                    ResizeTab tab, bool direct, int n, hipStream_t s, unsigned flags);
hipError_t launch_fill_u8(uint8_t* p, uint8_t v, size_t bytes, hipStream_t s);

}
```

backscrub_amd/csrc/kernels_seg.hip:

```cpp
#ifndef __HIPCC_RTC__
#include <hip/hip_runtime.h>
#endif
#ifndef BSX_SEG_RTC
#include "debug_switches.hpp"

#include <algorithm>
#include <cstdlib>

#include "kernels.hpp"
#include "mfma_tile.hpp"
#include "segments.hpp"
#endif

#if defined(BSX_SEG_RTC)
#define BSX_SEG_D(T, NAME) constexpr T d = kSeg##NAME; (void)d_rt
#elif defined(BSX_SEG_PROBE)
#define BSX_SEG_D(T, NAME) constexpr T d = kProbe##NAME; (void)d_rt
#else
#define BSX_SEG_D(T, NAME) const T& d = d_rt
#endif

namespace bsx {
#ifdef BSX_SEG_RTC
namespace segrtc {
// ... 74 lines not shown
constexpr int kGateStageFloats = kSegGateStageFloats;
__device__ __forceinline__ void seg_gate(const SegGate& gt, const float* __restrict__ fa, const float* __restrict__ w, float* scr, float* stage) {
  float* s_gate = scr + kScrGate;
  if (gt.timing_skip) { if (threadIdx.x < 16) s_gate[threadIdx.x] = 0.5f; __syncthreads(); return; }
  float* s_mean = scr + kScrGate + 16;
  float* s_hid = scr + kScrGate + 48;
  const int tid = threadIdx.x;
  const SegFc &f1 = gt.fc[0], &f2 = gt.fc[1];
  const int w1n = f1.Cin * f1.Cout, w2n = gt.n_fc == 2 ? f2.Cin * f2.Cout : 0;
  float* ps = stage;
  float* w1 = ps + 512;
  float* b1 = w1 + w1n;
  float* w2 = b1 + f1.Cout;
  float* b2 = w2 + w2n;
  {
    const int c = tid & 15, slice = tid >> 4;
    for (int k = 0; k < gt.n_parts; k++) {
      const float* src = fa + gt.part[k].off;
      float s = 0.f;
#pragma unroll 4
      for (int i = slice; i < gt.part[k].n; i += 16) s += src[(unsigned)(i * 16 + c)];
      ps[k * 256 + slice * 16 + c] = s;
    }
  }
  {
    const float* g1 = w + f1.w_off;
    const float* g2 = w + f2.w_off;
    for (int i = tid; i < w1n; i += kSegThreads) w1[i] = g1[(unsigned)i];
    for (int i = tid; i < w2n; i += kSegThreads) w2[i] = g2[(unsigned)i];
    if (tid < f1.Cout) b1[tid] = (w + f1.b_off)[(unsigned)tid];
    if (gt.n_fc == 2 && tid < f2.Cout) b2[tid] = (w + f2.b_off)[(unsigned)tid];
  }
  __syncthreads();
  const int Cm = gt.sum_parts ? 16 : 16 * gt.n_parts;
  if (tid < Cm) {
    float m = 0.f;
    for (int k = 0; k < gt.n_parts; k++) {
      if (!gt.sum_parts && (tid >> 4) != k) continue;
      float s = 0.f;
#pragma unroll
      for (int sl = 0; sl < 16; sl++) s += ps[k * 256 + sl * 16 + (tid & 15)];
      m += s / gt.part[k].hw;
    }
    s_mean[tid] = m;
  }
  __syncthreads();
  auto fc = [&](const SegFc& f, const float* x, const float* wl, const float* bl, float* y) {
    const int out = tid >> 3, ks = tid & 7, kper = f.Cin >> 3;
    float acc = 0.f;
    if (out < f.Cout)
      for (int j = 0; j < kper; j++) acc = fmaf(x[ks * kper + j], wl[out * f.Cin + ks * kper + j], acc);
    acc += dpp_quad(acc, 1);
    acc += dpp_quad(acc, 2);
    acc += __builtin_bit_cast(float, __builtin_amdgcn_update_dpp(0, __builtin_bit_cast(int, acc), 0x141, 0xf, 0xf, true));
    if (out < f.Cout && ks == 0) y[out] = sg_act(acc + bl[out], f.act);
  };
  fc(f1, s_mean, w1, b1, gt.n_fc == 1 ? s_gate : s_hid);
  __syncthreads();
  if (gt.n_fc == 2) {
    fc(f2, s_hid, w2, b2, s_gate);
    __syncthreads();
  }
}

template <int SHR>
__device__ __forceinline__ float dpp_row_shr(float v) {
  return __builtin_bit_cast(float, __builtin_amdgcn_update_dpp(0, __builtin_bit_cast(int, v), 0x110 + SHR, 0xf, 0xf, true));
}
template <int MODE>
__device__ __forceinline__ void wave_reduce16(float4 v, float* s_red, int wave, int lane) {
  if (MODE == 0) {
    v.x += dpp_row_shr<1>(v.x); v.y += dpp_row_shr<1>(v.y); v.z += dpp_row_shr<1>(v.z); v.w += dpp_row_shr<1>(v.w);
    v.x += dpp_row_shr<2>(v.x); v.y += dpp_row_shr<2>(v.y); v.z += dpp_row_shr<2>(v.z); v.w += dpp_row_shr<2>(v.w);
    v.x += dpp_row_shr<4>(v.x); v.y += dpp_row_shr<4>(v.y); v.z += dpp_row_shr<4>(v.z); v.w += dpp_row_shr<4>(v.w);
    v.x += dpp_row_shr<8>(v.x); v.y += dpp_row_shr<8>(v.y); v.z += dpp_row_shr<8>(v.z); v.w += dpp_row_shr<8>(v.w);
    const int li = lane & 15;
    if (li >= 12) st4(s_red + (wave * 4 + (15 - li)) * 16 + 4 * (lane >> 4), li == 15 ? v : f4zero());
  } else {
    v.x += dpp_row_shr<4>(v.x); v.y += dpp_row_shr<4>(v.y); v.z += dpp_row_shr<4>(v.z); v.w += dpp_row_shr<4>(v.w);
    v.x += dpp_row_shr<8>(v.x); v.y += dpp_row_shr<8>(v.y); v.z += dpp_row_shr<8>(v.z); v.w += dpp_row_shr<8>(v.w);
    if ((lane & 12) == 12) st4(s_red + (wave * 4 + (lane >> 4)) * 16 + 4 * (lane & 3), v);
  }
}
__device__ __forceinline__ void store_partials(const float* s_red, float* dst ) {
  if (threadIdx.x < 16) {
    float s = 0.f;
#pragma unroll
    for (int j = 0; j < 16; j++) s += s_red[j * 16 + threadIdx.x];
    dst[threadIdx.x] = s;
  }
}

__device__ __forceinline__ void up_axis(int o, float scale, bool half_pixel, int in_size, int* lo, int* hi, float* frac) {
  const float v = half_pixel ? __fadd_rn(__fmul_rn((float)o + 0.5f, scale), -0.5f) : __fmul_rn((float)o, scale);
  const float fl = floorf(v);
  *lo = max((int)fl, 0);
  *hi = min((int)ceilf(v), in_size - 1);
  *frac = v - (float)*lo;
}
__device__ __forceinline__ float up_scale(int in, int out, bool align) { return (align && out > 1) ? (float)(in - 1) / (float)(out - 1) : (float)in / (float)out; }

__device__ __forceinline__ float quad_reduce_scatter(float p0, float p1, float p2, float p3, int quad) {
  const bool b0 = quad & 1, b1 = quad & 2;
  const float klo = (b0 ? p1 : p0) + dpp_quad(b0 ? p0 : p1, 1);
  const float khi = (b0 ? p3 : p2) + dpp_quad(b0 ? p2 : p3, 1);
  return (b1 ? khi : klo) + dpp_quad(b1 ? klo : khi, 2);
}

typedef float f4v __attribute__((ext_vector_type(4)));
__device__ __forceinline__ f4v ldv(const float* p) { return *reinterpret_cast<const f4v*>(p); }
__device__ __forceinline__ f4v tov(float4 a) { f4v r = {a.x, a.y, a.z, a.w}; return r; }
__device__ __forceinline__ float4 tof4(f4v a) { return make_float4(a.x, a.y, a.z, a.w); }
__device__ __forceinline__ f4v dw3x3(const float* __restrict__ zt, int RWF, int row0, const int (&co)[3], const f4v (&wd)[9]) {
  f4v acc = {0.f, 0.f, 0.f, 0.f};
  const float* base = zt + row0 * RWF;
#pragma unroll
  for (int fy = 0; fy < 3; fy++)
#pragma unroll
    for (int fx = 0; fx < 3; fx++) acc = __builtin_elementwise_fma(ldv(base + fy * RWF + co[fx]), wd[fy * 3 + fx], acc);
  return acc;
}

__device__ __forceinline__ uint32_t seg_meet_val(float l0, float l1) {
  const float d = l1 - l0;
  if (fabsf(l0) <= 80.f && fabsf(l1) <= 80.f && fabsf(d) >= 1e-4f) return d > 0.f ? 0u : 255u;
  const float e0 = (float)exp((double)l0), e1 = (float)exp((double)l1);
  const float s = __fadd_rn(e0, e1);
  return __fdiv_rn(e0, s) < __fdiv_rn(e1, s) ? 0u : 255u;
}

__device__ __forceinline__ int wave_uniform(int v) { return __builtin_amdgcn_readfirstlane(v); }

struct RowTile { int row, ct; };
__device__ __forceinline__ RowTile row_tile(int t, int ctiles, unsigned m_ct) {
  RowTile r;
  r.row = (int)(((unsigned)t * m_ct) >> 16);
  r.ct = t - r.row * ctiles;
  return r;
}

#ifdef BSX_SEG_RTC
extern "C" __global__ __launch_bounds__(kSegThreads) void bsx_seg_head(
#else
template <bool STEM_HSWISH, bool H16, bool U8IN>
__global__ __launch_bounds__(kSegThreads) void seg_head_k(
#endif
    const SegHead d_rt, float* __restrict__ arena, long per_frame, const float* __restrict__ net_in,
                                                          const float* __restrict__ w, float in_scale, float in_offset, int n_frames) {
  BSX_SEG_D(SegHead, HEAD);
  unsigned f_, t_;
  xcd_frame_tile((unsigned)(d.tiles_y * d.tiles_x), (unsigned)n_frames, &f_, &t_);
  const int f = (int)f_, ty = (int)t_ / d.tiles_x, tx = (int)t_ - ty * d.tiles_x;
  const int r0 = ty * d.TR, c0 = tx * d.TC;
  const int AR = 2 * d.TR + 1, AC = 2 * d.TC + 1, ar0 = 2 * r0 - d.dw_pt, ac0 = 2 * c0 - d.dw_pl, RW = d.rw, ctiles = RW >> 4;
  const int IR = 2 * AR + 1, IC = 2 * AC + 1, ir0 = 2 * ar0 - d.stem_pt, ic0 = 2 * ac0 - d.stem_pl, rowf = IC * 3;
  float* fa = arena + (size_t)f * (size_t)per_frame;
  float* in_t = seg_smem;
  float* a_t = in_t + max(512, (IR * rowf + 3) & ~3);
  float* A_out = fa + d.a_off;
  float* b0_out = fa + d.b0_off;
  const int tid = threadIdx.x, lane = tid & 63, wave = wave_uniform(tid >> 6), li = lane & 15, g = lane >> 4, cq4 = 4 * g;

  if (d.dbg_skip & 8) {  } else
  if (U8IN) {
    const uint32_t* src = reinterpret_cast<const uint32_t*>(net_in) + (size_t)f * (size_t)(d.H0 * d.W0);
    const bool colok = lane < IC && ic0 + lane >= 0 && ic0 + lane < d.W0;
    const int gxc = min(max(ic0 + lane, 0), d.W0 - 1);
    uint32_t v[5];
    bool ok[5];
#pragma unroll
    for (int j = 0; j < 5; j++) {
      const int row = wave + 4 * j, gy = ir0 + row;
      ok[j] = row < IR && gy >= 0 && gy < d.H0 && colok;
// ... 34 lines not shown
  int koff[7];
  float ws[7];
#pragma unroll
  for (int s = 0; s < 7; s++) {
    const int k = 4 * s + g;
    const bool valid = k < 27;
    const int fy = k / 9, r9 = k - 9 * fy, fx = r9 / 3, ci = r9 - 3 * fx;
    koff[s] = valid ? fy * rowf + fx * 3 + ci : 0;
    ws[s] = valid ? (w + d.stem.w_off)[(unsigned)(k * d.stem.cout_pad + li)] : 0.f;
  }
  const float4 bias_s = ld4(w + d.stem.b_off + cq4);
  const Clamp cl_stem = clamp_of(d.stem.act), cl_pw = clamp_of(d.pw.act), cl_dw = clamp_of(d.dw.act);
  const int ntile = AR * ctiles;
  const int xe = li;
  __syncthreads();

  float* x_f = a_t;
  float wr[4];
  load_wtile(wr, w, d.pw, 0, li, g);
  const float4 bias_p = ld4(w + d.pw.b_off + cq4);
  float4 sumA = f4zero();
  auto stem_pw_epilogue = [&](const f4acc acc, const RowTile rt) {
    float4 v = acc_quad(acc);
    const int x2 = 16 * rt.ct + xe, gy = ar0 + rt.row, gx = ac0 + x2;
    v = f4add(v, bias_s);
    v = STEM_HSWISH ? hswish4(v) : clamp4(v, cl_stem);
    f4acc pa = {0.f, 0.f, 0.f, 0.f};
    if (!(d.dbg_skip & 2)) {
      pa = __builtin_amdgcn_mfma_f32_16x16x4f32(wr[0], v.x, pa, 0, 0, 0);
      pa = __builtin_amdgcn_mfma_f32_16x16x4f32(wr[1], v.y, pa, 0, 0, 0);
      pa = __builtin_amdgcn_mfma_f32_16x16x4f32(wr[2], v.z, pa, 0, 0, 0);
      pa = __builtin_amdgcn_mfma_f32_16x16x4f32(wr[3], v.w, pa, 0, 0, 0);
    }
    if (x2 < AC) {
      const bool row_owned = gy >= max(2 * r0, 0) && gy < min(2 * r0 + 2 * d.TR, d.H1);
      if (row_owned && gx >= 2 * c0 && gx < min(2 * c0 + 2 * d.TC, d.W1)) {
        stg4<H16>(A_out, (unsigned)((gy * d.W1 + gx) * 16 + cq4), v);
        sumA = f4add(sumA, v);
      }
      float4 xv = acc_quad(pa);
      const bool inside = gy >= 0 && gy < d.H1 && gx >= 0 && gx < d.W1;
      xv = inside ? clamp4(f4add(xv, bias_p), cl_pw) : f4zero();
      st4(x_f + (rt.row * AC + x2) * 16 + cq4, xv);
    }
  };
  for (int t = wave; t < ntile && !(d.dbg_skip & 1); t += 8) {
    const bool two = t + 4 < ntile;
    const RowTile r0t = row_tile(t, ctiles, d.m_ct), r1t = row_tile(two ? t + 4 : t, ctiles, d.m_ct);
    const float* base0 = in_t + (2 * r0t.row) * rowf + 6 * min(16 * r0t.ct + li, AC - 1);
    const float* base1 = in_t + (2 * r1t.row) * rowf + 6 * min(16 * r1t.ct + li, AC - 1);
    float av0[7], av1[7];
#pragma unroll
    for (int s7 = 0; s7 < 7; s7++) { av0[s7] = base0[koff[s7]]; av1[s7] = base1[koff[s7]]; }
    f4acc acc0 = {0.f, 0.f, 0.f, 0.f}, acc1 = {0.f, 0.f, 0.f, 0.f};
#pragma unroll
    for (int s7 = 0; s7 < 7; s7++) {
      acc0 = __builtin_amdgcn_mfma_f32_16x16x4f32(ws[s7], av0[s7], acc0, 0, 0, 0);
      acc1 = __builtin_amdgcn_mfma_f32_16x16x4f32(ws[s7], av1[s7], acc1, 0, 0, 0);
    }
    stem_pw_epilogue(acc0, r0t);
    if (two) stem_pw_epilogue(acc1, r1t);
  }
  const int quad = lane & 3, px = lane >> 2;
  f4v wd[9];
#pragma unroll
  for (int k = 0; k < 9; k++) wd[k] = ldv(w + d.dw.w_off + k * 16 + 4 * quad);
  const f4v bias_d = ldv(w + d.dw.b_off + 4 * quad);
  const int cox[3] = {(2 * px) * 16 + 4 * quad, (2 * px + 1) * 16 + 4 * quad, (2 * px + 2) * 16 + 4 * quad};
  __syncthreads();

  float4 sumB = f4zero();
  for (int py = wave; py < d.TR && !(d.dbg_skip & 4); py += 4) {
    if (r0 + py >= d.H2) break;
    if (px < d.TC && c0 + px < d.W2) {
      const float4 v = clamp4(tof4(dw3x3(x_f, AC * 16, 2 * py, cox, wd) + bias_d), cl_dw);
      stg4<H16>(b0_out, (unsigned)(((r0 + py) * d.W2 + c0 + px) * 16 + 4 * quad), v);
      sumB = f4add(sumB, v);
    }
  }
  float* s_red = in_t;
  wave_reduce16<0>(sumA, s_red, wave, lane);
  wave_reduce16<1>(sumB, s_red + 256, wave, lane);
  __syncthreads();
  store_partials(s_red, fa + d.part_a_off + (long)t_ * 16);
  store_partials(s_red + 256, fa + d.part_b0_off + (long)t_ * 16);
}

#ifdef BSX_SEG_RTC
extern "C" __global__ __launch_bounds__(kSegThreads) __attribute__((amdgpu_waves_per_eu(6, 6))) void bsx_seg_k2(
#else
template <bool H16>
__global__ __launch_bounds__(kSegThreads) __attribute__((amdgpu_waves_per_eu(6, 6))) void seg_k2_k(
#endif
    const SegK2 d_rt, float* __restrict__ arena, long per_frame, const float* __restrict__ w, int n_frames) {
  BSX_SEG_D(SegK2, K2);
  unsigned f_, t_;
  xcd_frame_tile((unsigned)(d.tiles_y * d.tiles_x), (unsigned)n_frames, &f_, &t_);
  const int f = (int)f_, ty = (int)t_ / d.tiles_x, tx = (int)t_ - ty * d.tiles_x;
  const int r0 = ty * d.TR, c0 = tx * d.TC;
  const int BR = 2 * d.TR + 1, BC = 2 * d.TC + 1, br0 = 2 * r0 - d.dw_pt, bc0 = 2 * c0 - d.dw_pl, RW = d.rw, ctiles = RW >> 4;
  float* fa = arena + (size_t)f * (size_t)per_frame;
  float* B_t = seg_smem + kScrFloats;
  float* x_t = B_t + BR * RW * 16;
  const float* b0_in = fa + d.b0_off;
  float* B_out = fa + d.B_off;
  float* c0_out = fa + d.c0_off;
  const int tid = threadIdx.x, lane = tid & 63, wave = wave_uniform(tid >> 6), li = lane & 15, g = lane >> 4, cq4 = 4 * g;
  const int ntile = BR * ctiles, xe = li;
  const int la = col_a(li, g), lb = col_b(li, g, RW >> 1);
  constexpr int kB0 = 6;
  float4 b0v[kB0];
#pragma unroll
  for (int j = 0; j < kB0; j++) {
    const int t = wave + 4 * j;
    b0v[j] = f4zero();
    if (t < ntile) {
      const RowTile rt = row_tile(t, ctiles, d.m_ct);
      const int gy = br0 + rt.row, gx = bc0 + 16 * rt.ct + li;
      if (gy >= 0 && gy < d.H2 && gx >= 0 && gx < d.W2) b0v[j] = ldg4<H16>(b0_in, (unsigned)((gy * d.W2 + gx) * 16 + 4 * g));
    }
  }
  seg_gate(d.gate, fa, w, seg_smem, B_t);
  const float4 sv = ld4(seg_smem + kScrGate + 4 * g);
  float wr[4];
  load_wtile(wr, w, d.pw_a, 0, li, g);
  const float4 bias_a = ld4(w + d.pw_a.b_off + cq4);
  const Clamp cl_a = clamp_of(d.pw_a.act), cl_b = clamp_of(d.pw_b.act), cl_dw = clamp_of(d.dw.act);

  float4 sumB = f4zero();
#pragma unroll
  for (int j = 0; j < kB0; j++) {
    const int t = wave + 4 * j;
    if (t >= ntile) break;
    const RowTile rt = row_tile(t, ctiles, d.m_ct);
    float4 a = b0v[j];
    a = make_float4(__fmul_rn(a.x, sv.x), __fmul_rn(a.y, sv.y), __fmul_rn(a.z, sv.z), __fmul_rn(a.w, sv.w));
    const f4acc acc = mma16(a, wr);
    float4 v = acc_quad(acc);
    const int x2 = 16 * rt.ct + xe, hy = br0 + rt.row, hx = bc0 + x2;
    if (x2 < BC) {
      v = clamp4(f4add(v, bias_a), cl_a);
      st4(B_t + (rt.row * RW + 16 * rt.ct) * 16 + la, v);
      const bool row_owned = hy >= max(2 * r0, 0) && hy < min(2 * r0 + 2 * d.TR, d.H2);
      if (row_owned && hx >= 2 * c0 && hx < min(2 * c0 + 2 * d.TC, d.W2)) {
        stg4<H16>(B_out, (unsigned)((hy * d.W2 + hx) * 16 + cq4), v);
        sumB = f4add(sumB, v);
      }
    }
  }
  float* s_red = seg_smem + kScrRed;
  wave_reduce16<0>(sumB, s_red, wave, lane);
  __syncthreads();
  store_partials(s_red, fa + d.part_B_off + (long)t_ * 16);

  const int C = d.dw.C, ngrp = (C + 15) >> 4, quad = lane & 3, px = lane >> 2;
  const int cox[3] = {col_b(2 * px, quad, RW >> 1), col_b(2 * px + 1, quad, RW >> 1), col_b(2 * px + 2, quad, RW >> 1)};
  for (int grp = 0; grp < ngrp && !(d.dbg_skip & 2); grp++) {
    load_wtile(wr, w, d.pw_b, 16 * grp, li, g);
    const float4 bias_b = ld4(w + d.pw_b.b_off + 16 * grp + cq4);
    for (int t = wave; t < ntile; t += 4) {
      const RowTile rt = row_tile(t, ctiles, d.m_ct);
      const f4acc acc = mma16(ld4(B_t + (rt.row * RW + 16 * rt.ct) * 16 + la), wr);
      float4 v = acc_quad(acc);
      const int x2 = 16 * rt.ct + xe, hy = br0 + rt.row, hx = bc0 + x2;
      if (x2 < BC) {
        const bool inside = hy >= 0 && hy < d.H2 && hx >= 0 && hx < d.W2;
        v = inside ? clamp4(f4add(v, bias_b), cl_b) : f4zero();
        st4(x_t + (rt.row * RW + 8 * rt.ct) * 16 + lb, v);
      }
    }
    const int ch = 16 * grp + 4 * quad;
    f4v wd[9];
    f4v bias_d = {0.f, 0.f, 0.f, 0.f};
    if (ch < C) {
#pragma unroll
      for (int k = 0; k < 9; k++) wd[k] = ldv(w + d.dw.w_off + (unsigned)(k * C + ch));
      bias_d = ldv(w + d.dw.b_off + ch);
    }
    __syncthreads();
    if (ch < C && px < d.TC && c0 + px < d.W3)
      for (int py = wave; py < d.TR && r0 + py < d.H3; py += 4) {
        const float4 v = clamp4(tof4(dw3x3(x_t, RW * 16, 2 * py, cox, wd) + bias_d), cl_dw);
        stg4<H16>(c0_out, (unsigned)(((r0 + py) * d.W3 + c0 + px) * C + ch), v);
      }
    __syncthreads();
  }
}

constexpr int kGatedRows = 5;
constexpr int kLoStride = kSegLoStride;
struct GatedPre { float4 s[kGatedRows]; int ly0, lx0, LC; };
template <bool H16>
__device__ __forceinline__ GatedPre gated_prefetch(const float* __restrict__ skip, const float* __restrict__ lo, int H, int W, int HL, int WL, bool half_pixel,
                                                   float hs, float wsc, int r0, int c0, int ZH, int ZC, float* l_t) {
  const int tid = threadIdx.x, lane = tid & 63, wave = wave_uniform(tid >> 6), li = lane & 15, g = lane >> 4;
  GatedPre pre;
  const int ix = c0 - 1 + li;
  const bool col_in = li < ZC && ix >= 0 && ix < W;
#pragma unroll
  for (int j = 0; j < kGatedRows; j++) {
    const int zy = wave + 4 * j, iy = r0 - 1 + zy;
    pre.s[j] = f4zero();
    if (zy < ZH && iy >= 0 && iy < H && col_in) pre.s[j] = ldg4<H16>(skip, (unsigned)((iy * W + ix) * 16 + 4 * g));
  }
  int ly0, ly1, lx0, lx1, t0, t1;
  float fr;
// ... 25 lines not shown
  const float4 bias = ld4(w + pw.b_off + cq4);
  const float4 gv = ld4(s_gate + 4 * g);
  const Clamp cl = clamp_of(pw.act);
  const int ix = c0 - 1 + li;
  int x0, x1;
  float dx;
  up_axis(min(max(ix, 0), W - 1), wsc, half_pixel, WL, &x0, &x1, &dx);
  const int xo0 = col_l(x0 - pre.lx0, g), xo1 = col_l(x1 - pre.lx0, g);
  const int xe = li;
  const bool ecol_in = xe < ZC && ix >= 0 && ix < W;
#pragma unroll
  for (int j = 0; j < kGatedRows; j++) {
    const int zy = wave + 4 * j, iy = r0 - 1 + zy;
    if (zy >= ZH) break;
    const bool row_in = iy >= 0 && iy < H;
    int y0, y1;
    float dy;
    up_axis(min(max(iy, 0), H - 1), hs, half_pixel, HL, &y0, &y1, &dy);
    const float* l0 = l_t + (y0 - pre.ly0) * pre.LC * kLoStride;
    const float* l1 = l_t + (y1 - pre.ly0) * pre.LC * kLoStride;
    const float4 ta = ld4(l0 + xo0), tb = ld4(l1 + xo0), tc = ld4(l0 + xo1), td = ld4(l1 + xo1);
    const float w00 = (1.f - dy) * (1.f - dx), w10 = dy * (1.f - dx), w01 = (1.f - dy) * dx, w11 = dy * dx;
    const float4 sk = pre.s[j];
    float4 a;
    a.x = fmaf(sk.x, gv.x, fmaf(td.x, w11, fmaf(tc.x, w01, fmaf(tb.x, w10, ta.x * w00))));
    a.y = fmaf(sk.y, gv.y, fmaf(td.y, w11, fmaf(tc.y, w01, fmaf(tb.y, w10, ta.y * w00))));
    a.z = fmaf(sk.z, gv.z, fmaf(td.z, w11, fmaf(tc.z, w01, fmaf(tb.z, w10, ta.z * w00))));
    a.w = fmaf(sk.w, gv.w, fmaf(td.w, w11, fmaf(tc.w, w01, fmaf(tb.w, w10, ta.w * w00))));
    const f4acc acc = mma16(a, wr);
    float4 v = acc_quad(acc);
    v = (ecol_in && row_in) ? clamp4(f4add(v, bias), cl) : f4zero();
    if (xe < ZC) st4(z_t + zy * 256 + col_a(xe, g), v);
  }
}

#ifdef BSX_SEG_RTC
extern "C" __global__ __launch_bounds__(kSegThreads) void bsx_seg_k3(
#else
template <bool H16>
__global__ __launch_bounds__(kSegThreads) void seg_k3_k(
#endif
    const SegK3 d_rt, float* __restrict__ arena, long per_frame, const float* __restrict__ w, int n_frames) {
  BSX_SEG_D(SegK3, K3);
  unsigned f_, t_;
  xcd_frame_tile((unsigned)(d.tiles_y * d.tiles_x), (unsigned)n_frames, &f_, &t_);
  const int f = (int)f_, ty = (int)t_ / d.tiles_x, tx = (int)t_ - ty * d.tiles_x;
  const int r0 = ty * d.TR, c0 = tx * d.TC, ZH = d.TR + 2, ZC = d.TC + 2;
  float* fa = arena + (size_t)f * (size_t)per_frame;
  float* z_t = seg_smem + kScrFloats;
  float* l_t = z_t + ZH * 256;
  float* lo_out = fa + d.lo_off;
  const int tid = threadIdx.x, lane = tid & 63, wave = wave_uniform(tid >> 6), li = lane & 15, g = lane >> 4, cq4 = 4 * g;
  const GatedPre pre = gated_prefetch<H16>(fa + d.skip_off, fa + d.lo2_off, d.H2, d.W2, d.HL, d.WL, d.half_pixel != 0, d.hs, d.ws, r0, c0, ZH, ZC, l_t);
  if (tid < 16) seg_smem[kScrGate + tid] = fa[d.g_off + tid];
  __syncthreads();
  gated_compute(pre, l_t, d.H2, d.W2, d.HL, d.WL, d.half_pixel != 0, d.hs, d.ws, seg_smem + kScrGate, d.pw1, w, r0, c0, ZH, ZC, z_t);
  const int pc = min(li, 13);
  const int coz[3] = {col_a(pc, g), col_a(pc + 1, g), col_a(pc + 2, g)};
  f4v wd[9];
#pragma unroll
  for (int k = 0; k < 9; k++) wd[k] = ldv(w + d.dw.w_off + k * 16 + cq4);
  const f4v bias_d = ldv(w + d.dw.b_off + cq4);
  const Clamp cl_dw = clamp_of(d.dw.act), cl_2 = clamp_of(d.pw2.act);
  float wr[4];
  load_wtile(wr, w, d.pw2, 0, li, g);
  const float4 bias2 = ld4(w + d.pw2.b_off + cq4);
  __syncthreads();
  float4 sum = f4zero();
  const int xe = li;
  for (int py = wave; py < d.TR && r0 + py < d.H2; py += 4) {
    const f4v zc = ldv(z_t + (py + 1) * 256 + coz[1]);
    const float4 dv = clamp4(tof4(dw3x3(z_t, 256, py, coz, wd) + bias_d), cl_dw);
    const f4acc acc = mma16(f4add(dv, tof4(zc)), wr);
    float4 v = acc_quad(acc);
    if (xe < d.TC && c0 + xe < d.W2) {
      v = clamp4(f4add(v, bias2), cl_2);
      stg4<H16>(lo_out, (unsigned)(((r0 + py) * d.W2 + c0 + xe) * 16 + cq4), v);
      sum = f4add(sum, v);
    }
  }
  float* s_red = seg_smem + kScrRed;
  wave_reduce16<0>(sum, s_red, wave, lane);
  __syncthreads();
  store_partials(s_red, fa + d.part_lo_off + (long)t_ * 16);
}

#ifdef BSX_SEG_RTC
extern "C" __global__ __launch_bounds__(kSegThreads) __attribute__((amdgpu_waves_per_eu(5, 5))) void bsx_seg_tail(
#else
template <int CO, bool LOGITS, bool SIGMOID, bool H16>
__global__ __launch_bounds__(kSegThreads) __attribute__((amdgpu_waves_per_eu(5, 5))) void seg_tail_k(
#endif
    const SegTail d_rt, float* __restrict__ arena, long per_frame, float* __restrict__ net_out,
                                                          uint8_t* __restrict__ ofinal, const float* __restrict__ w, int n_frames) {
  BSX_SEG_D(SegTail, TAIL);
  unsigned f_, t_;
  xcd_frame_tile((unsigned)(d.tiles_y * d.tiles_x), (unsigned)n_frames, &f_, &t_);
  const int f = (int)f_, ty = (int)t_ / d.tiles_x, tx = (int)t_ - ty * d.tiles_x;
  const int r0 = ty * d.TR, c0 = tx * d.TC, ZH = d.TR + 2, ZC = d.TC + 2;
  float* fa = arena + (size_t)f * (size_t)per_frame;
  float* z_t = seg_smem + kScrFloats;
  float* l_t = z_t + max(ZH * 256, kGateStageFloats);
  uint8_t* of = ofinal + (size_t)f * (size_t)(d.H0 * d.W0);
  float* no = net_out + (size_t)f * (size_t)(d.H0 * d.W0 * CO);
  const int tid = threadIdx.x, lane = tid & 63, wave = wave_uniform(tid >> 6), li = lane & 15, g = lane >> 4, cq4 = 4 * g;
  const int fy = g >> 1, fx = g & 1, ix = c0 + li;
  const GatedPre pre = gated_prefetch<H16>(fa + d.skip_off, fa + d.lo_off, d.H1, d.W1, d.HL, d.WL, d.half_pixel != 0, d.hs, d.ws, r0, c0, ZH, ZC, l_t);
  constexpr int kRowsB = 5;
  const bool lane_on = li < d.TC && ix < d.W1;
  uint8_t prev[kRowsB];
  if (!LOGITS) {
#pragma unroll
    for (int j = 0; j < kRowsB; j++) {
      const int py = wave + 4 * j, iy = r0 + py;
      prev[j] = 0;
      if (py < d.TR && iy < d.H1 && lane_on) prev[j] = of[(unsigned)((2 * iy + fy) * d.W0 + 2 * ix + fx)];
    }
  }
  if (d.pre_gate_off >= 0) {
    if (tid < 16) seg_smem[kScrGate + tid] = fa[d.pre_gate_off + tid];
    __syncthreads();
  } else seg_gate(d.gate, fa, w, seg_smem, z_t);
  if (!(d.dbg_skip & 1)) gated_compute(pre, l_t, d.H1, d.W1, d.HL, d.WL, d.half_pixel != 0, d.hs, d.ws, seg_smem + kScrGate, d.pw, w, r0, c0, ZH, ZC, z_t);
  if (d.dbg_skip & 2) return;
  f4v wd[9];
#pragma unroll
  for (int k = 0; k < 9; k++) wd[k] = ldv(w + d.dw.w_off + k * 16 + cq4);
  const f4v bias_d = ldv(w + d.dw.b_off + cq4);
  float wtr[4];
#pragma unroll
  for (int r = 0; r < 4; r++) wtr[r] = (li & 3) < CO ? w[d.tc_w_off + (unsigned)((((li >> 2) * CO + (li & 3)) * 16) + cq4 + r)] : 0.f;
  float bt[CO];
#pragma unroll
  for (int oc = 0; oc < CO; oc++) bt[oc] = w[d.tc_b_off + oc];
  const Clamp cl_dw = clamp_of(d.dw.act);
  const int pc = min(li, 13);
  const int coz[3] = {col_a(pc, g), col_a(pc + 1, g), col_a(pc + 2, g)};
  __syncthreads();
#pragma unroll
  for (int j = 0; j < kRowsB; j++) {
    const int py = wave + 4 * j, iy = r0 + py;
    if (py >= d.TR || iy >= d.H1) break;
    const f4v zc = ldv(z_t + (py + 1) * 256 + coz[1]);
    const float4 t4 = f4add(clamp4(tof4(dw3x3(z_t, 256, py, coz, wd) + bias_d), cl_dw), tof4(zc));
    const f4acc acc = mma16(t4, wtr);
    if (lane_on) {
      float o[CO];
#pragma unroll
      for (int oc = 0; oc < CO; oc++) {
        o[oc] = bt[oc] + acc[oc];
        if (SIGMOID) o[oc] = sigmoid1(o[oc]);
      }
      const int oy = 2 * iy + fy, ox = 2 * ix + fx;
      const unsigned opix = (unsigned)(oy * d.W0 + ox);
      if (LOGITS) {
#pragma unroll
        for (int oc = 0; oc < CO; oc++) no[opix * CO + oc] = o[oc];
      } else {
        uint32_t val;
        if (CO == 2) val = seg_meet_val(o[0], o[CO - 1]);
        else val = ((double)o[0] > 0.65) ? 0u : 255u;
        of[opix] = (uint8_t)((val & 0xE0u) | ((uint32_t)prev[j] >> 3));
      }
    }
  }
}

#ifndef BSX_SEG_RTC
__global__ __launch_bounds__(kSegThreads) void seg_gate_k(const SegGate gt, float* __restrict__ arena, long per_frame, const float* __restrict__ w, long long out_off) {
  float* fa = arena + (size_t)blockIdx.x * (size_t)per_frame;
  seg_gate(gt, fa, w, seg_smem, seg_smem + kScrFloats);
  if (threadIdx.x < 16) fa[out_off + threadIdx.x] = seg_smem[kScrGate + threadIdx.x];
}

template <class K>
hipError_t allow_lds(K kernel, int lds_bytes) {
  return hipFuncSetAttribute(reinterpret_cast<const void*>(kernel), hipFuncAttributeMaxDynamicSharedMemorySize, lds_bytes);
}
#endif

}

#ifndef BSX_SEG_RTC
hipError_t seg_prepare() {
  const int full = 160 * 1024;
  hipError_t e = hipSuccess;
  auto one = [&](auto k) { if (e == hipSuccess) e = allow_lds(k, full); };
  one(seg_head_k<true, false, false>); one(seg_head_k<false, false, false>); one(seg_head_k<true, true, false>); one(seg_head_k<false, true, false>);
  one(seg_head_k<true, false, true>); one(seg_head_k<false, false, true>); one(seg_head_k<true, true, true>); one(seg_head_k<false, true, true>);
  one(seg_k2_k<false>); one(seg_k2_k<true>); one(seg_k3_k<false>); one(seg_k3_k<true>);
  one(seg_tail_k<1, false, true, false>); one(seg_tail_k<1, true, true, false>); one(seg_tail_k<1, false, false, false>); one(seg_tail_k<1, true, false, false>);
  one(seg_tail_k<2, false, false, false>); one(seg_tail_k<2, true, false, false>);
  one(seg_tail_k<1, false, true, true>); one(seg_tail_k<1, true, true, true>); one(seg_tail_k<1, false, false, true>); one(seg_tail_k<1, true, false, true>);
  one(seg_tail_k<2, false, false, true>); one(seg_tail_k<2, true, false, true>);
  return e;
}

static int xcd_frames(int n) { static const bool on = !(BSX_DBG_ENV("BSX_XCD_TILES") && atoi(BSX_DBG_ENV("BSX_XCD_TILES")) == 0); return on ? n : 0; }

hipError_t launch_seg_head(const SegHead& d, float* arena, long per_frame, const void* net_in, const float* weights, int n, hipStream_t s, bool h16, bool u8, float in_scale,
                           float in_offset) {
  const dim3 grid((unsigned)(d.tiles_y * d.tiles_x) * (unsigned)n);
  const size_t lds = (size_t)d.lds_floats * sizeof(float);
  const bool hs = d.stem.act == kActHswish;
  const float* in = static_cast<const float*>(net_in);
  if (u8 && 2 * (2 * d.TC + 1) + 1 > 64) return hipErrorInvalidValue;
#define BSX_HEAD(HS, H, U) seg_head_k<HS, H, U><<<grid, kSegThreads, lds, s>>>(d, arena, per_frame, in, weights, in_scale, in_offset, xcd_frames(n))
  if (hs) { if (h16) { if (u8) BSX_HEAD(true, true, true); else BSX_HEAD(true, true, false); } else { if (u8) BSX_HEAD(true, false, true); else BSX_HEAD(true, false, false); } }
  else { if (h16) { if (u8) BSX_HEAD(false, true, true); else BSX_HEAD(false, true, false); } else { if (u8) BSX_HEAD(false, false, true); else BSX_HEAD(false, false, false); } }
#undef BSX_HEAD
  return hipGetLastError();
}
hipError_t launch_seg_k2(const SegK2& d, float* arena, long per_frame, const float* weights, int n, hipStream_t s, bool h16) {
  const dim3 grid((unsigned)(d.tiles_y * d.tiles_x) * (unsigned)n);
  if (h16) seg_k2_k<true><<<grid, kSegThreads, (size_t)d.lds_floats * sizeof(float), s>>>(d, arena, per_frame, weights, xcd_frames(n));
  else seg_k2_k<false><<<grid, kSegThreads, (size_t)d.lds_floats * sizeof(float), s>>>(d, arena, per_frame, weights, xcd_frames(n));
  return hipGetLastError();
}
hipError_t launch_seg_k3(const SegK3& d, float* arena, long per_frame, const float* weights, int n, hipStream_t s, bool h16) {
  const dim3 grid((unsigned)(d.tiles_y * d.tiles_x) * (unsigned)n);
  if (h16) seg_k3_k<true><<<grid, kSegThreads, (size_t)d.lds_floats * sizeof(float), s>>>(d, arena, per_frame, weights, xcd_frames(n));
  else seg_k3_k<false><<<grid, kSegThreads, (size_t)d.lds_floats * sizeof(float), s>>>(d, arena, per_frame, weights, xcd_frames(n));
  return hipGetLastError();
}
template <bool H16>
static hipError_t launch_seg_tail_t(const SegTail& d, float* arena, long per_frame, float* net_out, uint8_t* ofinal, const float* weights, bool logits, int n, hipStream_t s) {
  const dim3 grid((unsigned)(d.tiles_y * d.tiles_x) * (unsigned)n);
  static const int wgs_cap = BSX_DBG_ENV("BSX_SEG_TAIL_WGS") ? atoi(BSX_DBG_ENV("BSX_SEG_TAIL_WGS")) : 0;
  size_t lds = (size_t)d.lds_floats * sizeof(float);
  if (wgs_cap > 0) lds = std::max(lds, (size_t)(160 * 1024 / (wgs_cap + 1) + 256));
  const bool sig = d.act3 == kActSigmoid;
  if (d.Co == 2 && !sig) {
    if (logits) seg_tail_k<2, true, false, H16><<<grid, kSegThreads, lds, s>>>(d, arena, per_frame, net_out, ofinal, weights, xcd_frames(n));
    else seg_tail_k<2, false, false, H16><<<grid, kSegThreads, lds, s>>>(d, arena, per_frame, net_out, ofinal, weights, xcd_frames(n));
  } else if (d.Co == 1 && sig) {
    if (logits) seg_tail_k<1, true, true, H16><<<grid, kSegThreads, lds, s>>>(d, arena, per_frame, net_out, ofinal, weights, xcd_frames(n));
    else seg_tail_k<1, false, true, H16><<<grid, kSegThreads, lds, s>>>(d, arena, per_frame, net_out, ofinal, weights, xcd_frames(n));
  } else if (d.Co == 1) {
    if (logits) seg_tail_k<1, true, false, H16><<<grid, kSegThreads, lds, s>>>(d, arena, per_frame, net_out, ofinal, weights, xcd_frames(n));
    else seg_tail_k<1, false, false, H16><<<grid, kSegThreads, lds, s>>>(d, arena, per_frame, net_out, ofinal, weights, xcd_frames(n));
  } else {
    return hipErrorInvalidValue;
  }
  return hipGetLastError();
}
hipError_t launch_seg_gate(const SegGate& gt, float* arena, long per_frame, const float* weights, long long out_off, int n, hipStream_t s) {
  seg_gate_k<<<n, kSegThreads, (size_t)(kSegScratchFloats + kSegGateStageFloats) * sizeof(float), s>>>(gt, arena, per_frame, weights, out_off);
  return hipGetLastError();
}
hipError_t launch_seg_tail(const SegTail& d, float* arena, long per_frame, float* net_out, uint8_t* ofinal, const float* weights, bool logits, int n, hipStream_t s, bool h16) {
  return h16 ? launch_seg_tail_t<true>(d, arena, per_frame, net_out, ofinal, weights, logits, n, s) : launch_seg_tail_t<false>(d, arena, per_frame, net_out, ofinal, weights, logits, n, s);
}

#endif

}
```

backscrub_amd/csrc/plan.cpp:

```cpp
#include "debug_switches.hpp"
#include "plan.hpp"
#include "gen_seg.hpp"
#include "gen_mid.hpp"

#include <algorithm>
#include <cmath>
#include <cstdio>
#include <cstdlib>
#include <cstring>
#include <map>

namespace bsx {
namespace {

void conv_geometry(int in, int k, int s, int d, bool same, int* out, int* pad) {
  int eff = (k - 1) * d + 1;
  *out = same ? (in + s - 1) / s : (in + s - eff) / s;
  int total = (*out - 1) * s + eff - in;
  *pad = total > 0 ? total / 2 : 0;
}

uint16_t f32_to_f16_rn(float f) {
  uint32_t x; memcpy(&x, &f, 4);
  const uint32_t sign = (x >> 16) & 0x8000u;
// ... 532 lines not shown
  if (!(pwb.kind == StepKind::PwConv && pwb.in0 == B && pwb.Cin == 16 && pwb.cout_pad % 16 == 0 && pwb.residual < 0 && pwb.in_scale < 0 && pwb.in2 < 0 &&
        uses_of(pwb.out) == 1 && pwb.Cout % 4 == 0)) return seg_fail(7);
  if (!(is_dw3(kdw, 2) && kdw.in0 == pwb.out && kdw.residual < 0)) return seg_fail(8);
  const int c0 = kdw.out;
  const Step &tr = S[NS - 7], &tg = S[NS - 6], &tf1 = S[NS - 5], &tf2 = S[NS - 4], &tpw = S[NS - 3], &tdw = S[NS - 2], &ttc = S[NS - 1];
  if (!(tr.kind == StepKind::Resize && tr.Cin == 16 && tr.OH == dims(A, 1) && tr.OW == dims(A, 2))) return seg_fail(9);
  const int lo = tr.in0, up = tr.out;
  auto pools = [](const Step& q, int a, int b) { return q.kind == StepKind::Gap && q.concat_in.size() == 2 && ((q.concat_in[0] == a && q.concat_in[1] == b) || (q.gap_sum && q.concat_in[0] == b && q.concat_in[1] == a)); };
  if (!(pools(tg, A, up) && is_fc_step(tf1) && tf1.in0 == tg.out &&
        is_fc_step(tf2) && tf2.in0 == tf1.out && tf2.Cout == 16)) return seg_fail(10);
  if (!(is_pw16(tpw) && tpw.in0 == A && tpw.in_scale == tf2.out && tpw.in2 == up && tpw.residual < 0)) return seg_fail(11);
  if (!(is_dw3(tdw, 1) && tdw.in0 == tpw.out && tdw.residual == tpw.out && tdw.Cout == 16 && tdw.pad_t == 1 && tdw.pad_l == 1)) return seg_fail(12);
  if (!(ttc.kind == StepKind::TConv && ttc.in0 == tdw.out && ttc.kh == 2 && ttc.kw == 2 && ttc.Cin == 16 && (ttc.Cout == 1 || ttc.Cout == 2) && ttc.out == g.output)) return seg_fail(13);
  if (uses_of(A) != 3 || uses_of(up) != 2 || uses_of(tpw.out) != 2 || uses_of(tdw.out) != 1 || uses_of(tf2.out) != 1) return seg_fail(14);
  if (!resize_weights_uniform(tr.H, tr.OH, tr.align_corners, tr.half_pixel) || !resize_weights_uniform(tr.W, tr.OW, tr.align_corners, tr.half_pixel)) return seg_fail(15);
  const Step &kr = S[NS - 14], &kg = S[NS - 13], &kf1 = S[NS - 12], &kf2 = S[NS - 11], &kp1 = S[NS - 10], &kd = S[NS - 9], &kp2 = S[NS - 8];
  if (!(kr.kind == StepKind::Resize && kr.Cin == 16 && kr.OH == dims(B, 1) && kr.OW == dims(B, 2))) return seg_fail(16);
  const int lo2 = kr.in0, up2 = kr.out;
  if (!(pools(kg, B, up2) && is_fc_step(kf1) && kf1.in0 == kg.out &&
        is_fc_step(kf2) && kf2.in0 == kf1.out && kf2.Cout == 16)) return seg_fail(17);
  if (!(is_pw16(kp1) && kp1.in0 == B && kp1.in_scale == kf2.out && kp1.in2 == up2 && kp1.residual < 0)) return seg_fail(18);
  if (!(is_dw3(kd, 1) && kd.in0 == kp1.out && kd.residual == kp1.out && kd.Cout == 16 && kd.pad_t == 1 && kd.pad_l == 1)) return seg_fail(19);
  if (!(is_pw16(kp2) && kp2.in0 == kd.out && kp2.out == lo && kp2.residual < 0 && kp2.in_scale < 0 && kp2.in2 < 0)) return seg_fail(20);
  if (uses_of(B) != 3 || uses_of(up2) != 2 || uses_of(kp1.out) != 2 || uses_of(kd.out) != 1 || uses_of(kf2.out) != 1 || uses_of(lo) != 1 || uses_of(lo2) != 1) return seg_fail(21);
  if (!resize_weights_uniform(kr.H, kr.OH, kr.align_corners, kr.half_pixel) || !resize_weights_uniform(kr.W, kr.OW, kr.align_corners, kr.half_pixel)) return seg_fail(22);
  if (uses_of(c0) != 1) return seg_fail(23);
  auto clampish = [](int a) { return a == kActNone || a == kActRelu || a == kActRelu6; };
  if (!(clampish(stem.act) || stem.act == kActHswish) || !(ttc.act == kActNone || ttc.act == kActSigmoid) || (ttc.act == kActSigmoid && ttc.Cout != 1)) return seg_fail(34);
  for (const Step* q : {&hpw, &hdw, &pwa, &pwb, &kdw, &kp1, &kd, &kp2, &tpw, &tdw}) if (!clampish(q->act)) return seg_fail(35);

  size_t top = plan->arena_floats_per_stream;
  auto reserve = [&](size_t floats) { size_t at = top; top += (floats + 63) / 64 * 64; return (long long)at; };
  auto synth = [&](const char* name, int n, int C) {
    TensorInfo t; t.dims[0] = 1; t.dims[1] = n; t.dims[2] = 1; t.dims[3] = C; t.shape = {1, n, 1, C}; t.name = name;
    g.tensors.push_back(t);
    plan->tensor_off.push_back(-1);
    return (int)g.tensors.size() - 1;
  };
  SegPlan sp;
  int tgt[8] = {4, 14, 4, 7, 16, 14, 18, 14};
  if (const char* e = BSX_DBG_ENV("BSX_SEG_TILES")) sscanf(e, "%d,%d,%d,%d,%d,%d,%d,%d", &tgt[0], &tgt[1], &tgt[2], &tgt[3], &tgt[4], &tgt[5], &tgt[6], &tgt[7]);
  auto split = [&](int extent, int target, int* tile, int* n) { *n = tiles_for(extent, std::max(1, target)); *tile = (extent + *n - 1) / *n; };

  SegHead& h = sp.head;
  h.H0 = stem.H; h.W0 = stem.W; h.H1 = stem.OH; h.W1 = stem.OW; h.H2 = hdw.OH; h.W2 = hdw.OW;
  h.stem_pt = stem.pad_t; h.stem_pl = stem.pad_l; h.dw_pt = hdw.pad_t; h.dw_pl = hdw.pad_l;
  h.stem = conv_w(stem); h.pw = conv_w(hpw); h.dw = dw_w(hdw);
  split(h.H2, tgt[0], &h.TR, &h.tiles_y); split(h.W2, tgt[1], &h.TC, &h.tiles_x);
  h.lds_floats = seg_head_lds_floats(h);
  h.rw = seg_row_width(2 * h.TC + 1); h.m_ct = (65536u + (unsigned)(h.rw / 16) - 1) / (unsigned)(h.rw / 16);
  if (h.TR > 4 || h.TC > 15 || (4 * h.TC + 3) * 3 > 192) return seg_fail(30);
  SegK2& k2 = sp.k2;
  k2.H2 = hdw.OH; k2.W2 = hdw.OW; k2.H3 = kdw.OH; k2.W3 = kdw.OW; k2.dw_pt = kdw.pad_t; k2.dw_pl = kdw.pad_l;
  k2.pw_a = conv_w(pwa); k2.pw_b = conv_w(pwb); k2.dw = dw_w(kdw);
  split(k2.H3, tgt[2], &k2.TR, &k2.tiles_y); split(k2.W3, tgt[3], &k2.TC, &k2.tiles_x);
  k2.lds_floats = seg_k2_lds_floats(k2);
  k2.rw = seg_row_width(2 * k2.TC + 1); k2.m_ct = (65536u + (unsigned)(k2.rw / 16) - 1) / (unsigned)(k2.rw / 16);
  if (k2.TC > 15 || ((2 * k2.TR + 1) * (k2.rw / 16) + 3) / 4 > 6) return seg_fail(31);
  SegK3& k3 = sp.k3;
  k3.H2 = kp1.OH; k3.W2 = kp1.OW; k3.HL = kr.H; k3.WL = kr.W; k3.half_pixel = kr.half_pixel; k3.align_corners = kr.align_corners;
  k3.pw1 = conv_w(kp1); k3.pw2 = conv_w(kp2); k3.dw = dw_w(kd);
  split(k3.H2, tgt[4], &k3.TR, &k3.tiles_y); split(k3.W2, tgt[5], &k3.TC, &k3.tiles_x);
  k3.hs = seg_up_scale(k3.HL, k3.H2, k3.align_corners != 0); k3.ws = seg_up_scale(k3.WL, k3.W2, k3.align_corners != 0);
  if (!BSX_DBG_ENV("BSX_SEG_LO_WORST")) k3.lo_floats = seg_lo_window_floats(k3.H2, k3.W2, k3.HL, k3.WL, k3.half_pixel != 0, k3.align_corners != 0, k3.TR, k3.TC, k3.tiles_y, k3.tiles_x);
  k3.lds_floats = seg_k3_lds_floats(k3);
  if (k3.TC > 14 || k3.TR > 18) return seg_fail(32);
  SegTail& tl = sp.tail;
  tl.H1 = tpw.OH; tl.W1 = tpw.OW; tl.HL = tr.H; tl.WL = tr.W; tl.H0 = ttc.OH; tl.W0 = ttc.OW; tl.half_pixel = tr.half_pixel; tl.align_corners = tr.align_corners;
  tl.pw = conv_w(tpw); tl.dw = dw_w(tdw); tl.tc_w_off = (long long)ttc.w_off; tl.tc_b_off = (long long)ttc.b_off; tl.Co = ttc.Cout; tl.act3 = ttc.act;
  split(tl.H1, tgt[6], &tl.TR, &tl.tiles_y); split(tl.W1, tgt[7], &tl.TC, &tl.tiles_x);
  tl.hs = seg_up_scale(tl.HL, tl.H1, tl.align_corners != 0); tl.ws = seg_up_scale(tl.WL, tl.W1, tl.align_corners != 0);
  if (!BSX_DBG_ENV("BSX_SEG_LO_WORST")) tl.lo_floats = seg_lo_window_floats(tl.H1, tl.W1, tl.HL, tl.WL, tl.half_pixel != 0, tl.align_corners != 0, tl.TR, tl.TC, tl.tiles_y, tl.tiles_x);
  tl.lds_floats = seg_tail_lds_floats(tl);
  if (tl.TC > 14 || tl.TR > 18) return seg_fail(33);
  const int lds_cap = 160 * 256;
  if (h.lds_floats > lds_cap || k2.lds_floats > lds_cap || k3.lds_floats > lds_cap || tl.lds_floats > lds_cap) return seg_fail(24);
  if (ttc.OH != 2 * tpw.OH || ttc.OW != 2 * tpw.OW || h.H2 != k3.H2 || h.W2 != k3.W2) return seg_fail(25);
  if (h.tiles_y * h.tiles_x > 1024 || k2.tiles_y * k2.tiles_x > 1024 || k3.tiles_y * k3.tiles_x > 1024) return seg_fail(26);

  const int pA = synth("partials(A)", h.tiles_y * h.tiles_x, 16), pb0 = synth("partials(b0)", h.tiles_y * h.tiles_x, 16);
  const int pB = synth("partials(B)", k2.tiles_y * k2.tiles_x, 16), plo = synth("partials(lo)", k3.tiles_y * k3.tiles_x, 16);
  const int pgt = BSX_DBG_ENV("BSX_SEG_NO_GATE_KERNEL") ? -1 : synth("gate(tail)", 1, 16);
  if (pgt >= 0) plan->tensor_off[pgt] = reserve(16);
  for (int t : {A, b0, B, c0, lo2, lo, kf2.out, pA, pb0, pB, plo}) plan->tensor_off[t] = reserve(g.tensors[t].elems());
  for (int t : {hpw.out, g1.out, f1a.out, f1b.out, pwb.out, up2, kg.out, kf1.out, kp1.out, kd.out, up, tg.out, tf1.out, tf2.out, tpw.out, tdw.out})
    if (t != g.output) plan->tensor_off[t] = -1;
  plan->arena_floats_per_stream = top;

  h.a_off = plan->tensor_off[A]; h.b0_off = plan->tensor_off[b0]; h.part_a_off = plan->tensor_off[pA]; h.part_b0_off = plan->tensor_off[pb0];
  k2.b0_off = plan->tensor_off[b0]; k2.B_off = plan->tensor_off[B]; k2.c0_off = plan->tensor_off[c0]; k2.part_B_off = plan->tensor_off[pB];
  k2.gate.n_parts = 1; k2.gate.n_fc = 2; k2.gate.sum_parts = 0;
  k2.gate.part[0].off = plan->tensor_off[pb0]; k2.gate.part[0].n = h.tiles_y * h.tiles_x; k2.gate.part[0].C = 16; k2.gate.part[0].hw = (float)(h.H2 * h.W2);
  k2.gate.fc[0] = fc_w(f1a); k2.gate.fc[1] = fc_w(f1b);
  k3.skip_off = plan->tensor_off[B]; k3.lo2_off = plan->tensor_off[lo2]; k3.g_off = plan->tensor_off[kf2.out]; k3.lo_off = plan->tensor_off[lo];
  k3.part_lo_off = plan->tensor_off[plo];
  tl.skip_off = plan->tensor_off[A]; tl.lo_off = plan->tensor_off[lo];
  tl.gate.n_parts = 2; tl.gate.n_fc = 2; tl.gate.sum_parts = tg.gap_sum ? 1 : 0;
  tl.gate.part[0].off = plan->tensor_off[pA]; tl.gate.part[0].n = h.tiles_y * h.tiles_x; tl.gate.part[0].C = 16; tl.gate.part[0].hw = (float)(h.H1 * h.W1);
  tl.gate.part[1].off = plan->tensor_off[plo]; tl.gate.part[1].n = k3.tiles_y * k3.tiles_x; tl.gate.part[1].C = 16; tl.gate.part[1].hw = (float)(k3.H2 * k3.W2);
  tl.gate.fc[0] = fc_w(tf1); tl.gate.fc[1] = fc_w(tf2);
  if (BSX_DBG_ENV("BSX_SEG_GATE_SKIP")) k2.gate.timing_skip = tl.gate.timing_skip = 1;
  if (const char* e = BSX_DBG_ENV("BSX_SEG_SKIP")) sscanf(e, "%d,%d,%d,%d", &h.dbg_skip, &k2.dbg_skip, &k3.dbg_skip, &tl.dbg_skip);
  tl.pre_gate_off = pgt >= 0 ? plan->tensor_off[pgt] : -1;
  if (tl.gate.fc[0].Cin != (tl.gate.sum_parts ? 16 : 32) || k2.gate.fc[0].Cin != 16) return seg_fail(27);

  std::vector<Step> mid(S.begin() + 9, S.begin() + (NS - 14));
  Step gate = kg;
  gate.concat_in = {B, lo2};
  gate.in0 = B;
  gate.label += "*";
  mid.push_back(gate); mid.push_back(kf1); mid.push_back(kf2);
  std::map<int, int> part_n, part_hw;
  part_n[B] = k2.tiles_y * k2.tiles_x; part_hw[B] = k2.H2 * k2.W2;
  const long B_real = plan->tensor_off[B];
  plan->tensor_off[B] = plan->tensor_off[pB];
  build_frame_program(g, plan, mid, {c0, B, lo2, kf2.out}, part_n, part_hw);
  plan->tensor_off[B] = B_real;
  if (plan->program.empty()) return seg_fail(28);
  sp.on = true;
  plan->seg = sp;
#ifdef BSX_DEBUG_SWITCHES
  if (const char* path = BSX_DBG_ENV("BSX_SEG_DUMP")) {
    if (FILE* f = fopen(path, "w")) { fputs(seg_constants_text(sp, "kProbe").c_str(), f); fclose(f); }
  }
#endif
  char line[256];
  plan->seg_text.clear();
  auto add = [&](const char* name, int TR, int TC, int ty, int tx, int lds) {
    snprintf(line, sizeof line, "segment %-5s tile %dx%d, %dx%d tiles per frame, LDS %.1f KiB\n", name, TR, TC, ty, tx, lds / 256.0);
    plan->seg_text += line;
  };
  add("head", h.TR, h.TC, h.tiles_y, h.tiles_x, h.lds_floats); add("k2", k2.TR, k2.TC, k2.tiles_y, k2.tiles_x, k2.lds_floats);
  add("k3", k3.TR, k3.TC, k3.tiles_y, k3.tiles_x, k3.lds_floats); add("tail", tl.TR, tl.TC, tl.tiles_y, tl.tiles_x, tl.lds_floats);
  return true;
}


MidGeometry mid_geometry_default() {
  static const MidGeometry geo = [] {
    MidGeometry m{kFrameThreads, kLdsTotalFloats};
    if (const char* e = BSX_DBG_ENV("BSX_MID_LANES")) { const int v = atoi(e); if (v == 512 || v == 1024) m.lanes = v; }
    if (const char* e = BSX_DBG_ENV("BSX_MID_LDS_KB")) { const int v = atoi(e); if (v >= 64 && v <= 160) m.lds_floats = v * 256; }
    return m;
  }();
  return geo;
}

bool build_plan(const Graph& g_in, Plan* plan, std::string* err, bool reuse_arena, bool segments) {
  auto fail = [&](const std::string& m) { if (err) *err = m; return false; };
  { const MidGeometry geo = mid_geometry_default(); plan->mid_lanes = geo.lanes; plan->lds_total_floats = geo.lds_floats; }
  Graph g = g_in;
  int NT = (int)g.tensors.size();
  const int NN = (int)g.nodes.size();

  std::vector<std::vector<int>> users(NT);
  for (int i = 0; i < NN; i++) for (int t : g.nodes[i].inputs) if (t >= 0 && !g.tensors[t].is_const) users[t].push_back(i);
  auto single_user = [&](int t) -> int { return (t != g.output && users[t].size() == 1) ? users[t][0] : -1; };

  std::vector<char> fused(NN, 0);
  std::vector<Step> steps;
  std::vector<float>& W = plan->weights;
  W.clear();
  auto align_w = [&]() { while (W.size() % 4) W.push_back(0.f); };

  for (int i = 0; i < NN; i++) {
    if (fused[i]) continue;
    const Node& n = g.nodes[i];
    const TensorInfo& out_t = g.tensors[n.output];
    Step st;
    st.last_node = n.index;
    auto T = [&](int k) -> const TensorInfo& { return g.tensors[n.inputs[k]]; };

    auto chain_epilogue = [&](int cur) -> int {
      for (;;) {
        int u = single_user(cur);
        if (u < 0 || fused[u]) break;
        const Node& y = g.nodes[u];
        if (is_unary(y.type) && st.act == kActNone && st.residual < 0) {
          st.act = unary_act(y.type); fused[u] = 1; cur = y.output; st.last_node = y.index; continue;
        }
        if (y.type == OpType::Add && y.act == kActNone && st.residual < 0 && y.inputs.size() == 2) {
          int other = y.inputs[0] == cur ? y.inputs[1] : y.inputs[0];
          if (other >= 0 && other != cur && !g.tensors[other].is_const && same_dims(g.tensors[other], g.tensors[cur])) {
            st.residual = other; fused[u] = 1; cur = y.output; st.last_node = y.index; continue;
          }
        }
// ... 490 lines not shown
```

backscrub_amd/csrc/segments.hpp:

```cpp
#pragma once
#ifndef BSX_SEG_RTC
#include <algorithm>
#include <cmath>
#include <cstdint>
#endif

namespace bsx {

struct SegConvW { long long w_off = 0, b_off = 0; int Cin = 0, Cout = 0, cout_pad = 0, act = 0; };
struct SegDwW { long long w_off = 0, b_off = 0; int C = 0, act = 0; };
struct SegFc { long long w_off = 0, b_off = 0; int Cin = 0, Cout = 0, act = 0; };
struct SegPart { long long off = 0; int n = 0, C = 0; float hw = 1.f; };
struct SegGate {
  int n_parts = 0, sum_parts = 0, n_fc = 0;
  int timing_skip = 0;
  SegPart part[2];
  SegFc fc[2];
};

constexpr int kSegThreads = 256;
constexpr int kSegMaxC = 16;

struct SegHead {
  int H0 = 0, W0 = 0, H1 = 0, W1 = 0, H2 = 0, W2 = 0;
  int stem_pt = 0, stem_pl = 0, dw_pt = 0, dw_pl = 0;
  SegConvW stem, pw;
  SegDwW dw;
  long long a_off = 0, b0_off = 0, part_a_off = 0, part_b0_off = 0;
  int TR = 0, TC = 0, tiles_y = 0, tiles_x = 0;
  int lds_floats = 0;
  int dbg_skip = 0;
  int rw = 0;
  unsigned m_ct = 0;
};

struct SegK2 {
  int H2 = 0, W2 = 0, H3 = 0, W3 = 0;
  int dw_pt = 0, dw_pl = 0;
  SegGate gate;
  SegConvW pw_a, pw_b;
  SegDwW dw;
  long long b0_off = 0, B_off = 0, c0_off = 0, part_B_off = 0;
  int TR = 0, TC = 0, tiles_y = 0, tiles_x = 0;
  int lds_floats = 0;
  int dbg_skip = 0;
  int rw = 0;
  unsigned m_ct = 0;
};

struct SegK3 {
  int H2 = 0, W2 = 0, HL = 0, WL = 0;
  int half_pixel = 0, align_corners = 0;
  SegConvW pw1, pw2;
  SegDwW dw;
  long long skip_off = 0, lo2_off = 0, g_off = 0, lo_off = 0, part_lo_off = 0;
  int TR = 0, TC = 0, tiles_y = 0, tiles_x = 0;
  int lds_floats = 0;
  int lo_floats = 0;
  float hs = 0.f, ws = 0.f;
  int dbg_skip = 0;
};

struct SegTail {
  int H1 = 0, W1 = 0, HL = 0, WL = 0, H0 = 0, W0 = 0;
  int half_pixel = 0, align_corners = 0;
  SegGate gate;
  SegConvW pw;
  SegDwW dw;
  long long tc_w_off = 0, tc_b_off = 0;
  int Co = 0, act3 = 0, model_type = 0;
  long long skip_off = 0, lo_off = 0;
  long long pre_gate_off = -1;
  int TR = 0, TC = 0, tiles_y = 0, tiles_x = 0;
  int lds_floats = 0;
  int lo_floats = 0;
  float hs = 0.f, ws = 0.f;
  int dbg_skip = 0;
};

constexpr int kSegLoStride = 16;
constexpr int kSegLoTileFloats = 12 * 16 * kSegLoStride;
constexpr int kSegScratchFloats = 640;
constexpr int kSegGateStageFloats = 512 + 2 * (32 * 32 + 32);
#ifndef BSX_SEG_RTC
inline int seg_row_width(int cols) { return (cols + 15) / 16 * 16; }
inline int seg_head_lds_floats(const SegHead& d) {
  const int AR = 2 * d.TR + 1, AC = 2 * d.TC + 1, IR = 2 * AR + 1, IC = 2 * AC + 1;
  const int win = (IR * IC * 3 + 3) & ~3;
  return (win > 512 ? win : 512) + AR * AC * 16;
}
inline int seg_k2_lds_floats(const SegK2& d) { const int v = 2 * (2 * d.TR + 1) * seg_row_width(2 * d.TC + 1) * 16; return kSegScratchFloats + (v > kSegGateStageFloats ? v : kSegGateStageFloats); }
inline void seg_up_axis(int o, float scale, bool half_pixel, int in_size, int* lo, int* hi) {
  const float v = half_pixel ? ((float)o + 0.5f) * scale + -0.5f : (float)o * scale;
  const float fl = std::floor(v);
  *lo = std::max((int)fl, 0);
  *hi = std::min((int)std::ceil(v), in_size - 1);
}
inline float seg_up_scale(int in, int out, bool align) { return (align && out > 1) ? (float)(in - 1) / (float)(out - 1) : (float)in / (float)out; }
inline int seg_lo_window_floats(int H, int W, int HL, int WL, bool half_pixel, bool align, int TR, int TC, int tiles_y, int tiles_x) {
  const float hs = seg_up_scale(HL, H, align), ws = seg_up_scale(WL, W, align);
  int lr = 1, lc = 1, a, b, c, e;
  for (int ty = 0; ty < tiles_y; ty++) {
    const int r0 = ty * TR;
    seg_up_axis(std::max(r0 - 1, 0), hs, half_pixel, HL, &a, &b);
    seg_up_axis(std::min(r0 + TR, H - 1), hs, half_pixel, HL, &c, &e);
    lr = std::max(lr, e - a + 1);
  }
  for (int tx = 0; tx < tiles_x; tx++) {
    const int c0 = tx * TC;
    seg_up_axis(std::max(c0 - 1, 0), ws, half_pixel, WL, &a, &b);
    seg_up_axis(std::min(c0 + TC, W - 1), ws, half_pixel, WL, &c, &e);
    lc = std::max(lc, e - a + 1);
  }
  const int need = (lr + 1) * (lc + 1) * kSegLoStride;
  return need < kSegLoTileFloats ? need : kSegLoTileFloats;
}
inline int seg_k3_lds_floats(const SegK3& d) { return kSegScratchFloats + (d.TR + 2) * 256 + (d.lo_floats > 0 ? d.lo_floats : kSegLoTileFloats); }
inline int seg_tail_lds_floats(const SegTail& d) { const int v = (d.TR + 2) * 256; return kSegScratchFloats + (v > kSegGateStageFloats ? v : kSegGateStageFloats) + (d.lo_floats > 0 ? d.lo_floats : kSegLoTileFloats); }
#endif

struct SegPlan {
  bool on = false;
  SegHead head;
  SegK2 k2;
  SegK3 k3;
  SegTail tail;
};

}
```

include/bsx.h:

```cpp
#ifndef BSX_H_
#define BSX_H_

#include <stddef.h>
#include <stdint.h>

#ifndef BSX_API
#define BSX_API __attribute__((visibility("default")))
#endif

#ifdef __cplusplus
extern "C" {
#endif

typedef struct bsx_ctx bsx_ctx;

typedef void (*bsx_debug_fn)(void* caller_ctx, const char* msg);
typedef void (*bsx_stage_fn)(void* caller_ctx);

enum {
  BSX_OK = 0,
  BSX_EINVAL = -1,
  BSX_EMODEL = -2,
  BSX_EDEVICE = -3,
  BSX_ESIZE = -4
// ... 18 lines not shown

BSX_API const char* bsx_version(void);

BSX_API int bsx_device_count(void);

BSX_API bsx_ctx* bsx_new(const char* model_path, size_t threads, size_t width, size_t height,
                 int n_streams, int device,
                 bsx_debug_fn ondebug, bsx_stage_fn onprep, bsx_stage_fn oninfer, bsx_stage_fn onmask,
                 void* caller_ctx);

BSX_API void bsx_delete(bsx_ctx* ctx);

BSX_API int bsx_get_info(const bsx_ctx* ctx, bsx_info* out);

BSX_API const char* bsx_last_error(const bsx_ctx* ctx);

BSX_API int bsx_reset(bsx_ctx* ctx, void* stream);

BSX_API int bsx_process_host(bsx_ctx* ctx, int stream_idx, const uint8_t* h_bgr, size_t bgr_stride,
                     uint8_t* h_mask, size_t mask_stride);

BSX_API int bsx_process_batch(bsx_ctx* ctx, const uint8_t* d_frames, int n, uint8_t* d_masks, void* stream);

BSX_API uint8_t* bsx_masks_device(bsx_ctx* ctx);

BSX_API int bsx_composite_batch(bsx_ctx* ctx, const uint8_t* d_bg, size_t bg_frame_stride,
                        const uint8_t* d_frames, const uint8_t* d_masks, uint8_t* d_out, int n, void* stream);

BSX_API int bsx_step_batch(bsx_ctx* ctx, const uint8_t* d_frames, const uint8_t* d_bg, size_t bg_frame_stride,
                   uint8_t* d_out, int n, void* stream);

BSX_API int bsx_step_batch_yuyv(bsx_ctx* ctx, const uint8_t* d_frames, const uint8_t* d_bg, size_t bg_frame_stride,
                        uint8_t* d_out_yuyv, int n, void* stream);

#define BSX_STEP_YUYV 1u
#define BSX_STEP_FLIP_H 2u
#define BSX_STEP_FLIP_V 4u
#define BSX_STEP_NO_MASK 8u
#define BSX_STEP_YUYV_IN 16u
#define BSX_STEP_BGBLUR(ksize) (((unsigned)(ksize) & 255u) << 8)
BSX_API int bsx_step_batch_ex(bsx_ctx* ctx, const uint8_t* d_frames, const uint8_t* d_bg, size_t bg_frame_stride,
                      uint8_t* d_out, int n, void* stream, unsigned flags);

BSX_API int bsx_step_batch_pipelined(bsx_ctx* ctx, const uint8_t* d_frames, const uint8_t* d_bg, size_t bg_frame_stride,
                             uint8_t* d_out, int n, void* stream, unsigned flags);

BSX_API int bsx_step_batch_vcam(bsx_ctx* ctx, const uint8_t* d_frames, const uint8_t* d_bg, size_t bg_frame_stride,
                                uint8_t* d_out, int out_w, int out_h, int n, void* stream, unsigned flags);

BSX_API int bsx_resize_bgr(bsx_ctx* ctx, const uint8_t* d_src, int sw, int sh, uint8_t* d_dst, int dw, int dh, int n, void* stream);

BSX_API int bsx_bgr_to_yuyv(bsx_ctx* ctx, const uint8_t* d_bgr, uint8_t* d_yuyv, int w, int h, int n, void* stream);

BSX_API int bsx_yuyv_to_bgr(bsx_ctx* ctx, const uint8_t* d_yuyv, uint8_t* d_bgr, int w, int h, int n, void* stream);

BSX_API int bsx_flip_bgr(bsx_ctx* ctx, const uint8_t* d_src, uint8_t* d_dst, int w, int h, int n, int code, void* stream);

BSX_API int bsx_gaussian_blur_bgr(bsx_ctx* ctx, const uint8_t* d_src, uint8_t* d_dst, int w, int h, int n, int ksize, void* stream);

typedef struct bsx_background bsx_background;
BSX_API bsx_background* bsx_background_load(bsx_ctx* ctx, const char* path, int debug);
BSX_API bsx_background* bsx_background_from_frames(bsx_ctx* ctx, const uint8_t* h_bgr, int width, int height, int n_frames, double fps, int debug);
BSX_API void bsx_background_free(bsx_background* bg);
BSX_API int bsx_background_info(const bsx_background* bg, int* width, int* height, int* n_frames, double* fps, int* is_video);
BSX_API int bsx_background_grab(bsx_background* bg, int width, int height, uint8_t* d_bgr_out, void* stream);
BSX_API int bsx_media_decode(const char* path, int* width, int* height, double* fps, uint8_t** h_bgr, char* errbuf, size_t errcap);
BSX_API void bsx_media_free(uint8_t* h_bgr);

typedef struct bsx_live bsx_live;
BSX_API bsx_live* bsx_live_new(bsx_ctx* ctx);
BSX_API void bsx_live_delete(bsx_live* live);
BSX_API int bsx_live_set_input_frame(bsx_live* live, const uint8_t* h_bgr, size_t bgr_stride);
BSX_API int bsx_live_get_output_mask(bsx_live* live, uint8_t* h_mask, size_t mask_stride);
BSX_API int bsx_live_timings(const bsx_live* live, long* waitns, long* loopns);

BSX_API int bsx_debug_buffer(bsx_ctx* ctx, int which, void** d_ptr, size_t* bytes);
BSX_API int bsx_debug_run_stage(bsx_ctx* ctx, int stage, const uint8_t* d_frames, int n, void* stream);
BSX_API const char* bsx_plan_describe(bsx_ctx* ctx);
BSX_API long bsx_debug_tensor(bsx_ctx* ctx, int tensor_idx, float* h_out, long cap);
BSX_API long bsx_debug_tensor_of(bsx_ctx* ctx, int tensor_idx, int stream_idx, float* h_out, long cap);

BSX_API int bsx_debug_mask_tile_stats(bsx_ctx* ctx, int n, long* out4);

BSX_API int bsx_debug_program_timeline(bsx_ctx* ctx, int n, unsigned long long* ticks, int cap, void* stream);

BSX_API int bsx_debug_gauss_coeffs(int ksize, int shift, uint32_t* c4 , uint32_t* c2 );

BSX_API int bsx_model_describe(const char* model_path, char* buf, size_t cap);
BSX_API int bsx_model_precompile(const char* model_path, const char* arch, char* msg, size_t cap);
BSX_API long bsx_model_kernel_source(const char* model_path, char* buf, size_t cap);
BSX_API long bsx_model_seg_source(const char* model_path, char* buf, size_t cap);

typedef struct bsx_launch_stat {
  char name[64];
  double avg_ms;
  double bytes;
  double flops;
} bsx_launch_stat;

BSX_API int bsx_profile_batch(bsx_ctx* ctx, const uint8_t* d_frames, const uint8_t* d_bg, size_t bg_frame_stride, uint8_t* d_out,
                      int n, int iters, bsx_launch_stat* out, int cap, void* stream);

#ifdef __cplusplus
}
#endif
#endif
```

Before: 725,500.

## Fold tail gate computation into seg_k3 via last-arriving-block handoff

Removes the standalone seg_gate kernel launch between seg_k3 and seg_tail. Each seg_k3 block now writes its partial sums with agent-scope atomic stores and bumps a per-frame atomic counter. The last block to arrive for a frame computes the gate and writes it into the arena. An optional variant does the same for the head→k2 gate (env-gated, off by default), and the arena is zeroed at init so the counters start at zero. The cost is an atomic, a fence and a serial gate epilogue on one block per frame, and a larger minimum LDS size for k3 and head that could lower occupancy.

```diff
diff --git a/backscrub_amd/api.py b/backscrub_amd/api.py
--- a/backscrub_amd/api.py
+++ b/backscrub_amd/api.py
@@ -73,6 +73,7 @@
     ("bsx_model_seg_source", C.c_long, [C.c_char_p, C.c_char_p, C.c_size_t]),
     ("bsx_debug_tensor_of", C.c_long, [C.c_void_p, C.c_int, C.c_int, C.POINTER(C.c_float), C.c_long]),
     ("bsx_debug_mask_tile_stats", C.c_int, [C.c_void_p, C.c_int, C.POINTER(C.c_long)]),
+    ("bsx_debug_seg_gates", C.c_int, [C.c_void_p, C.c_int, C.POINTER(C.c_float)]),
     ("bsx_debug_program_timeline", C.c_int, [C.c_void_p, C.c_int, C.POINTER(C.c_ulonglong), C.c_int, C.c_void_p]),
     ("bsx_model_describe", C.c_int, [C.c_char_p, C.c_char_p, C.c_size_t]),
     ("bsx_profile_batch", C.c_int, [C.c_void_p, C.c_void_p, C.c_void_p, C.c_size_t, C.c_void_p, C.c_int, C.c_int, C.POINTER(LaunchStat), C.c_int, C.c_void_p]),
@@ -334,6 +335,12 @@
         _check(lib().bsx_debug_mask_tile_stats(self.h, n or self.n_streams, a), self.h, "bsx_debug_mask_tile_stats")
         return {"tiles": a[0], "uniform_255": a[1], "uniform_0": a[2], "general": a[3], "tile": "128x32"}
 
+    def seg_gates(self, n=None):
+        n = n or self.n_streams
+        a = np.empty((n, 4, 16), np.float32)
+        _check(lib().bsx_debug_seg_gates(self.h, n, a.ctypes.data_as(C.POINTER(C.c_float))), self.h, "bsx_debug_seg_gates")
+        return a[:, 0:2].copy(), a[:, 2:4].copy()
+
     def graph_tensor(self, idx, stream=None) -> np.ndarray:
         if stream is not None:
             n = lib().bsx_debug_tensor_of(self.h, idx, stream, None, 0)
diff --git a/backscrub_amd/csrc/bsx_api.hip b/backscrub_amd/csrc/bsx_api.hip
--- a/backscrub_amd/csrc/bsx_api.hip
+++ b/backscrub_amd/csrc/bsx_api.hip
@@ -6,6 +6,7 @@
 #include <cstdio>
 #include <cstdlib>
 #include <cstring>
+#include <limits>
 #include <map>
 #include <memory>
 #include <string>
@@ -235,6 +236,7 @@
   BSX_HIP(c, hipStreamCreateWithFlags(&c->own_stream, hipStreamNonBlocking));
   const size_t N = (size_t)c->n_streams;
   BSX_HIP(c, hipMalloc(&c->d_arena, c->plan.arena_floats_per_stream * N * sizeof(float)));
+  BSX_HIP(c, hipMemset(c->d_arena, 0, c->plan.arena_floats_per_stream * N * sizeof(float)));
   BSX_HIP(c, hipMalloc(&c->d_net_in, N * c->inW * c->inH * c->inC * sizeof(float)));
   BSX_HIP(c, hipMalloc(&c->d_net_in_u8, N * c->inW * c->inH * sizeof(uint32_t)));
   BSX_HIP(c, hipMalloc(&c->d_net_out, N * c->outW * c->outH * c->outC * sizeof(float)));
@@ -410,6 +412,8 @@
   return seg_launch(c->seg_fn[2], d.tiles_y * d.tiles_x, n, d.lds_floats, s, args);
 }
 
+bool seg_gate_launch(const SegPlan& sp) { return sp.tail.pre_gate_off >= 0 && sp.k3.pre_gate_off < 0; }
+
 int run_infer(bsx_ctx* c, int n, hipStream_t s, bool logits = true, int slot = 0) {
   bsx_roctx::Range range("bsx:network");
   if (c->use_program && c->plan.seg.on) {
@@ -419,7 +423,7 @@
     BSX_HIP(c, seg_k2(c, n, s));
     BSX_HIP(c, launch_program(c, n, s));
     BSX_HIP(c, seg_k3(c, n, s));
-    if (sp.tail.pre_gate_off >= 0) BSX_HIP(c, launch_seg_gate(sp.tail.gate, c->d_arena, pf, c->d_weights, sp.tail.pre_gate_off, n, s));
+    if (seg_gate_launch(sp)) BSX_HIP(c, launch_seg_gate(sp.tail.gate, c->d_arena, pf, c->d_weights, sp.tail.pre_gate_off, n, s));
     if (!logits) { const int frc = state_write_fence(c, s); if (frc) return frc; }
     BSX_HIP(c, seg_tail(c, c->d_ofinal + (size_t)slot * c->outW * c->outH, logits, n, s));
     return BSX_OK;
@@ -1028,7 +1032,7 @@
   const bool seg = c->use_program && c->plan.seg.on;
   const bool fused_decode = infer_decodes(c);
   const bool atail = argmax_tail(c);
-  const int n_net = c->use_program ? (seg ? (c->plan.seg.tail.pre_gate_off >= 0 ? 6 : 5) : 1) : (int)c->plan.steps.size();
+  const int n_net = c->use_program ? (seg ? (seg_gate_launch(c->plan.seg) ? 6 : 5) : 1) : (int)c->plan.steps.size();
   const bool fuse_tail = !c->onmask && !c->no_mask_blend_fusion &&
                          mask_blend_fusable(c->width, c->height, c->roi, d_bg, bg_stride, d_frames, d_out);
   const int L = 1 + n_net + (fused_decode ? 0 : 1) + (fuse_tail ? 1 : 2) + (fuse_tail ? 1 : 0);
@@ -1055,7 +1059,7 @@
       BSX_TIMED(seg_k2(c, n, s));
       BSX_TIMED(launch_program(c, n, s));
       BSX_TIMED(seg_k3(c, n, s));
-      if (sp.tail.pre_gate_off >= 0) BSX_TIMED(launch_seg_gate(sp.tail.gate, c->d_arena, pf, c->d_weights, sp.tail.pre_gate_off, n, s));
+      if (seg_gate_launch(sp)) BSX_TIMED(launch_seg_gate(sp.tail.gate, c->d_arena, pf, c->d_weights, sp.tail.pre_gate_off, n, s));
       BSX_TIMED(seg_tail(c, c->d_ofinal, !fused_decode, n, s));
     } else if (c->use_program)
       BSX_TIMED(launch_program(c, n, s));
@@ -1100,7 +1104,7 @@
     put(j++, "seg_k2", N * 4.0 * (eb0 + eb0 + ec0), N * 2.0 * macs(3, 8));
     put(j++, "frame_program", N * 4.0 * (ec0 + elo2) + 4.0 * c->plan.weights.size(), N * 2.0 * macs(9, NS - 11));
     put(j++, "seg_k3", N * 4.0 * (eb0 + elo2 + elo), N * 2.0 * macs(NS - 10, NS - 8));
-    if (sp.tail.pre_gate_off >= 0) put(j++, "seg_gate", N * 4.0 * (16.0 * (sp.tail.gate.part[0].n + sp.tail.gate.part[1].n) + 16.0), 0);
+    if (seg_gate_launch(sp)) put(j++, "seg_gate", N * 4.0 * (16.0 * (sp.tail.gate.part[0].n + sp.tail.gate.part[1].n) + 16.0), 0);
     put(j++, fused_decode ? "seg_tail+decode" : "seg_tail", N * (4.0 * (eA + elo) + (fused_decode ? 2.0 * c->outW * c->outH : 4.0 * eout)), N * 2.0 * macs(NS - 7, NS - 1));
   } else if (c->use_program) {
     double io = (double)c->inW * c->inH * c->inC + (double)c->outW * c->outH * c->outC;
@@ -1160,6 +1164,31 @@
   if (hipDeviceSynchronize() != hipSuccess || hipMemcpy(cls.data(), c->d_tile_class, cls.size(), hipMemcpyDeviceToHost) != hipSuccess) return BSX_EDEVICE;
   out4[3] = 0;
   for (uint8_t v : cls) out4[v == 1 ? 1 : (v == 2 ? 2 : 3)]++;
+  return BSX_OK;
+}
+
+int bsx_debug_seg_gates(bsx_ctx* c, int n, float* out) {
+  if (!c || !out || n <= 0 || n > c->n_streams || !c->use_program || !c->plan.seg.on) return BSX_EINVAL;
+  DeviceGuard guard(c->device);
+  const SegPlan& sp = c->plan.seg;
+  const long pf = (long)c->plan.arena_floats_per_stream;
+  std::vector<float> h((size_t)n * 64, std::numeric_limits<float>::quiet_NaN());
+  float* d = nullptr;
+  BSX_HIP(c, hipDeviceSynchronize());
+  BSX_HIP(c, hipMalloc(&d, (size_t)n * 32 * sizeof(float)));
+  hipError_t e = launch_seg_gate_to(sp.k2.gate, c->d_arena, pf, c->d_weights, d, 32, n, nullptr);
+  if (e == hipSuccess) e = launch_seg_gate_to(sp.tail.gate, c->d_arena, pf, c->d_weights, d + 16, 32, n, nullptr);
+  if (e == hipSuccess) e = hipDeviceSynchronize();
+  std::vector<float> rec((size_t)n * 32);
+  if (e == hipSuccess) e = hipMemcpy(rec.data(), d, rec.size() * sizeof(float), hipMemcpyDeviceToHost);
+  for (int i = 0; i < n && e == hipSuccess; i++) {
+    if (sp.k2.pre_gate_off >= 0) e = hipMemcpy(&h[(size_t)i * 64], c->d_arena + (size_t)i * pf + sp.k2.pre_gate_off, 16 * sizeof(float), hipMemcpyDeviceToHost);
+    if (e == hipSuccess && sp.tail.pre_gate_off >= 0) e = hipMemcpy(&h[(size_t)i * 64 + 16], c->d_arena + (size_t)i * pf + sp.tail.pre_gate_off, 16 * sizeof(float), hipMemcpyDeviceToHost);
+    std::copy(rec.begin() + (size_t)i * 32, rec.begin() + (size_t)i * 32 + 32, h.begin() + (size_t)i * 64 + 32);
+  }
+  (void)hipFree(d);
+  BSX_HIP(c, e);
+  std::copy(h.begin(), h.end(), out);
   return BSX_OK;
 }
 
diff --git a/backscrub_amd/csrc/gen_seg.cpp b/backscrub_amd/csrc/gen_seg.cpp
--- a/backscrub_amd/csrc/gen_seg.cpp
+++ b/backscrub_amd/csrc/gen_seg.cpp
@@ -35,15 +35,18 @@
   const SegHead& H = sp.head; const SegK2& K2 = sp.k2; const SegK3& K3 = sp.k3; const SegTail& T = sp.tail;
   P("// segment descriptors of the loaded graph as constants (gen_seg.cpp: seg_constants_text)\nconstexpr SegHead %sHEAD = [] { SegHead t{};\n", pre);
   P("  t.H0 = %d; t.W0 = %d; t.H1 = %d; t.W1 = %d; t.H2 = %d; t.W2 = %d; t.stem_pt = %d; t.stem_pl = %d; t.dw_pt = %d; t.dw_pl = %d;\n", H.H0, H.W0, H.H1, H.W1, H.H2, H.W2, H.stem_pt, H.stem_pl, H.dw_pt, H.dw_pl);
-  conv("stem", H.stem); conv("pw", H.pw); dw("dw", H.dw);
+  conv("stem", H.stem); conv("pw", H.pw); dw("dw", H.dw); gate("gate", H.gate);
+  P("  t.pre_gate_off = %lldll; t.cnt_off = %lldll;\n", H.pre_gate_off, H.cnt_off);
   P("  t.a_off = %lldll; t.b0_off = %lldll; t.part_a_off = %lldll; t.part_b0_off = %lldll; t.TR = %d; t.TC = %d; t.tiles_y = %d; t.tiles_x = %d; t.lds_floats = %d; t.rw = %d; t.m_ct = %uu;\n  return t; }();\n",
           H.a_off, H.b0_off, H.part_a_off, H.part_b0_off, H.TR, H.TC, H.tiles_y, H.tiles_x, H.lds_floats, H.rw, H.m_ct);
   P("constexpr SegK2 %sK2 = [] { SegK2 t{};\n  t.H2 = %d; t.W2 = %d; t.H3 = %d; t.W3 = %d; t.dw_pt = %d; t.dw_pl = %d;\n", pre, K2.H2, K2.W2, K2.H3, K2.W3, K2.dw_pt, K2.dw_pl);
   gate("gate", K2.gate); conv("pw_a", K2.pw_a); conv("pw_b", K2.pw_b); dw("dw", K2.dw);
+  P("  t.pre_gate_off = %lldll;\n", K2.pre_gate_off);
   P("  t.b0_off = %lldll; t.B_off = %lldll; t.c0_off = %lldll; t.part_B_off = %lldll; t.TR = %d; t.TC = %d; t.tiles_y = %d; t.tiles_x = %d; t.lds_floats = %d; t.rw = %d; t.m_ct = %uu;\n  return t; }();\n",
           K2.b0_off, K2.B_off, K2.c0_off, K2.part_B_off, K2.TR, K2.TC, K2.tiles_y, K2.tiles_x, K2.lds_floats, K2.rw, K2.m_ct);
   P("constexpr SegK3 %sK3 = [] { SegK3 t{};\n  t.H2 = %d; t.W2 = %d; t.HL = %d; t.WL = %d; t.half_pixel = %d; t.align_corners = %d;\n", pre, K3.H2, K3.W2, K3.HL, K3.WL, K3.half_pixel, K3.align_corners);
-  conv("pw1", K3.pw1); conv("pw2", K3.pw2); dw("dw", K3.dw);
+  conv("pw1", K3.pw1); conv("pw2", K3.pw2); dw("dw", K3.dw); gate("gate", K3.gate);
+  P("  t.pre_gate_off = %lldll; t.cnt_off = %lldll;\n", K3.pre_gate_off, K3.cnt_off);
   P("  t.skip_off = %lldll; t.lo2_off = %lldll; t.g_off = %lldll; t.lo_off = %lldll; t.part_lo_off = %lldll; t.TR = %d; t.TC = %d; t.tiles_y = %d; t.tiles_x = %d; t.lds_floats = %d; t.lo_floats = %d; t.hs = (float)%.9g; t.ws = (float)%.9g;\n  return t; }();\n",
           K3.skip_off, K3.lo2_off, K3.g_off, K3.lo_off, K3.part_lo_off, K3.TR, K3.TC, K3.tiles_y, K3.tiles_x, K3.lds_floats, K3.lo_floats, (double)K3.hs, (double)K3.ws);
   P("constexpr SegTail %sTAIL = [] { SegTail t{};\n  t.H1 = %d; t.W1 = %d; t.HL = %d; t.WL = %d; t.H0 = %d; t.W0 = %d; t.half_pixel = %d; t.align_corners = %d;\n", pre, T.H1, T.W1, T.HL, T.WL, T.H0, T.W0, T.half_pixel, T.align_corners);
diff --git a/backscrub_amd/csrc/kernels.hpp b/backscrub_amd/csrc/kernels.hpp
--- a/backscrub_amd/csrc/kernels.hpp
+++ b/backscrub_amd/csrc/kernels.hpp
@@ -38,6 +38,7 @@
 hipError_t launch_seg_k2(const SegK2& d, float* arena, long per_frame, const float* weights, int n, hipStream_t s, bool h16 = false);
 hipError_t launch_seg_k3(const SegK3& d, float* arena, long per_frame, const float* weights, int n, hipStream_t s, bool h16 = false);
 hipError_t launch_seg_gate(const SegGate& gt, float* arena, long per_frame, const float* weights, long long out_off, int n, hipStream_t s);
+hipError_t launch_seg_gate_to(const SegGate& gt, const float* arena, long per_frame, const float* weights, float* out, long out_stride, int n, hipStream_t s);
 hipError_t launch_seg_tail(const SegTail& d, float* arena, long per_frame, float* net_out, uint8_t* ofinal, const float* weights, bool logits, int n, hipStream_t s, bool h16 = false);
 
 struct ResizeTab {
diff --git a/backscrub_amd/csrc/kernels_seg.hip b/backscrub_amd/csrc/kernels_seg.hip
--- a/backscrub_amd/csrc/kernels_seg.hip
+++ b/backscrub_amd/csrc/kernels_seg.hip
@@ -180,13 +180,33 @@
     if ((lane & 12) == 12) st4(s_red + (wave * 4 + (lane >> 4)) * 16 + 4 * (lane & 3), v);
   }
 }
+template <bool WT = false>
 __device__ __forceinline__ void store_partials(const float* s_red, float* dst ) {
   if (threadIdx.x < 16) {
     float s = 0.f;
 #pragma unroll
     for (int j = 0; j < 16; j++) s += s_red[j * 16 + threadIdx.x];
-    dst[threadIdx.x] = s;
-  }
+    if (WT) __hip_atomic_store((__attribute__((address_space(1))) float*)dst + threadIdx.x, s, __ATOMIC_RELAXED, __HIP_MEMORY_SCOPE_AGENT);
+    else dst[threadIdx.x] = s;
+  }
+}
+
+constexpr int kScrFlag = kScrRed + 512;
+__device__ __forceinline__ bool seg_last_arriver(float* cnt_word, unsigned tiles, float* scr) {
+  asm volatile("s_waitcnt vmcnt(0)" ::: "memory");
+  __syncthreads();
+  int* s_flag = reinterpret_cast<int*>(scr + kScrFlag);
+  if (threadIdx.x == 0) {
+    const unsigned old = __builtin_amdgcn_atomic_inc32((__attribute__((address_space(1))) unsigned*)cnt_word, tiles - 1u, __ATOMIC_RELAXED, "agent");
+    const bool last = old == tiles - 1u;
+    if (last) {
+      __builtin_amdgcn_fence(__ATOMIC_ACQUIRE, "agent");
+      asm volatile("s_waitcnt vmcnt(0)" ::: "memory");
+    }
+    *s_flag = last ? 1 : 0;
+  }
+  __syncthreads();
+  return *s_flag != 0;
 }
 
 __device__ __forceinline__ void up_axis(int o, float scale, bool half_pixel, int in_size, int* lo, int* hi, float* frac) {
@@ -387,8 +407,12 @@
   wave_reduce16<0>(sumA, s_red, wave, lane);
   wave_reduce16<1>(sumB, s_red + 256, wave, lane);
   __syncthreads();
-  store_partials(s_red, fa + d.part_a_off + (long)t_ * 16);
-  store_partials(s_red + 256, fa + d.part_b0_off + (long)t_ * 16);
+  store_partials<true>(s_red, fa + d.part_a_off + (long)t_ * 16);
+  store_partials<true>(s_red + 256, fa + d.part_b0_off + (long)t_ * 16);
+  if (d.pre_gate_off >= 0 && seg_last_arriver(fa + d.cnt_off, (unsigned)(d.tiles_y * d.tiles_x), seg_smem)) {
+    seg_gate(d.gate, fa, w, seg_smem, seg_smem + kScrFloats);
+    if (tid < 16) fa[d.pre_gate_off + tid] = seg_smem[kScrGate + tid];
+  }
 }
 
 #ifdef BSX_SEG_RTC
@@ -425,8 +449,12 @@
       if (gy >= 0 && gy < d.H2 && gx >= 0 && gx < d.W2) b0v[j] = ldg4<H16>(b0_in, (unsigned)((gy * d.W2 + gx) * 16 + 4 * g));
     }
   }
-  seg_gate(d.gate, fa, w, seg_smem, B_t);
-  const float4 sv = ld4(seg_smem + kScrGate + 4 * g);
+  float4 sv;
+  if (d.pre_gate_off >= 0) sv = ld4(fa + d.pre_gate_off + 4 * g);
+  else {
+    seg_gate(d.gate, fa, w, seg_smem, B_t);
+    sv = ld4(seg_smem + kScrGate + 4 * g);
+  }
   float wr[4];
   load_wtile(wr, w, d.pw_a, 0, li, g);
   const float4 bias_a = ld4(w + d.pw_a.b_off + cq4);
@@ -618,7 +646,11 @@
   float* s_red = seg_smem + kScrRed;
   wave_reduce16<0>(sum, s_red, wave, lane);
   __syncthreads();
-  store_partials(s_red, fa + d.part_lo_off + (long)t_ * 16);
+  store_partials<true>(s_red, fa + d.part_lo_off + (long)t_ * 16);
+  if (d.pre_gate_off >= 0 && seg_last_arriver(fa + d.cnt_off, (unsigned)(d.tiles_y * d.tiles_x), seg_smem)) {
+    seg_gate(d.gate, fa, w, seg_smem, seg_smem + kScrFloats);
+    if (tid < 16) fa[d.pre_gate_off + tid] = seg_smem[kScrGate + tid];
+  }
 }
 
 #ifdef BSX_SEG_RTC
@@ -703,10 +735,11 @@
 }
 
 #ifndef BSX_SEG_RTC
-__global__ __launch_bounds__(kSegThreads) void seg_gate_k(const SegGate gt, float* __restrict__ arena, long per_frame, const float* __restrict__ w, long long out_off) {
-  float* fa = arena + (size_t)blockIdx.x * (size_t)per_frame;
+__global__ __launch_bounds__(kSegThreads) void seg_gate_k(const SegGate gt, const float* __restrict__ arena, long per_frame, const float* __restrict__ w, float* __restrict__ out,
+                                                          long out_stride) {
+  const float* fa = arena + (size_t)blockIdx.x * (size_t)per_frame;
   seg_gate(gt, fa, w, seg_smem, seg_smem + kScrFloats);
-  if (threadIdx.x < 16) fa[out_off + threadIdx.x] = seg_smem[kScrGate + threadIdx.x];
+  if (threadIdx.x < 16) out[(size_t)blockIdx.x * (size_t)out_stride + threadIdx.x] = seg_smem[kScrGate + threadIdx.x];
 }
 
 template <class K>
@@ -781,7 +814,10 @@
   return hipGetLastError();
 }
 hipError_t launch_seg_gate(const SegGate& gt, float* arena, long per_frame, const float* weights, long long out_off, int n, hipStream_t s) {
-  seg_gate_k<<<n, kSegThreads, (size_t)(kSegScratchFloats + kSegGateStageFloats) * sizeof(float), s>>>(gt, arena, per_frame, weights, out_off);
+  return launch_seg_gate_to(gt, arena, per_frame, weights, arena + out_off, per_frame, n, s);
+}
+hipError_t launch_seg_gate_to(const SegGate& gt, const float* arena, long per_frame, const float* weights, float* out, long out_stride, int n, hipStream_t s) {
+  seg_gate_k<<<n, kSegThreads, (size_t)(kSegScratchFloats + kSegGateStageFloats) * sizeof(float), s>>>(gt, arena, per_frame, weights, out, out_stride);
   return hipGetLastError();
 }
 hipError_t launch_seg_tail(const SegTail& d, float* arena, long per_frame, float* net_out, uint8_t* ofinal, const float* weights, bool logits, int n, hipStream_t s, bool h16) {
diff --git a/backscrub_amd/csrc/plan.cpp b/backscrub_amd/csrc/plan.cpp
--- a/backscrub_amd/csrc/plan.cpp
+++ b/backscrub_amd/csrc/plan.cpp
@@ -638,6 +638,8 @@
   const int pB = synth("partials(B)", k2.tiles_y * k2.tiles_x, 16), plo = synth("partials(lo)", k3.tiles_y * k3.tiles_x, 16);
   const int pgt = BSX_DBG_ENV("BSX_SEG_NO_GATE_KERNEL") ? -1 : synth("gate(tail)", 1, 16);
   if (pgt >= 0) plan->tensor_off[pgt] = reserve(16);
+  const bool handoff = !BSX_DBG_ENV("BSX_SEG_NO_HANDOFF"), k2_handoff = handoff && BSX_DBG_ENV("BSX_SEG_K2_HANDOFF");
+  const long long hand_cnt = handoff ? reserve(16) : -1, k2_gate = k2_handoff ? reserve(16) : -1;
   for (int t : {A, b0, B, c0, lo2, lo, kf2.out, pA, pb0, pB, plo}) plan->tensor_off[t] = reserve(g.tensors[t].elems());
   for (int t : {hpw.out, g1.out, f1a.out, f1b.out, pwb.out, up2, kg.out, kf1.out, kp1.out, kd.out, up, tg.out, tf1.out, tf2.out, tpw.out, tdw.out})
     if (t != g.output) plan->tensor_off[t] = -1;
@@ -658,6 +660,8 @@
   if (BSX_DBG_ENV("BSX_SEG_GATE_SKIP")) k2.gate.timing_skip = tl.gate.timing_skip = 1;
   if (const char* e = BSX_DBG_ENV("BSX_SEG_SKIP")) sscanf(e, "%d,%d,%d,%d", &h.dbg_skip, &k2.dbg_skip, &k3.dbg_skip, &tl.dbg_skip);
   tl.pre_gate_off = pgt >= 0 ? plan->tensor_off[pgt] : -1;
+  if (k2_handoff) { h.gate = k2.gate; h.cnt_off = hand_cnt; h.pre_gate_off = k2.pre_gate_off = k2_gate; }
+  if (handoff && tl.pre_gate_off >= 0) { k3.gate = tl.gate; k3.cnt_off = hand_cnt + 4; k3.pre_gate_off = tl.pre_gate_off; }
   if (tl.gate.fc[0].Cin != (tl.gate.sum_parts ? 16 : 32) || k2.gate.fc[0].Cin != 16) return seg_fail(27);
 
   std::vector<Step> mid(S.begin() + 9, S.begin() + (NS - 14));
diff --git a/backscrub_amd/csrc/segments.hpp b/backscrub_amd/csrc/segments.hpp
--- a/backscrub_amd/csrc/segments.hpp
+++ b/backscrub_amd/csrc/segments.hpp
@@ -27,6 +27,8 @@
   SegConvW stem, pw;
   SegDwW dw;
   long long a_off = 0, b0_off = 0, part_a_off = 0, part_b0_off = 0;
+  SegGate gate;
+  long long pre_gate_off = -1, cnt_off = -1;
   int TR = 0, TC = 0, tiles_y = 0, tiles_x = 0;
   int lds_floats = 0;
   int dbg_skip = 0;
@@ -41,6 +43,7 @@
   SegConvW pw_a, pw_b;
   SegDwW dw;
   long long b0_off = 0, B_off = 0, c0_off = 0, part_B_off = 0;
+  long long pre_gate_off = -1;
   int TR = 0, TC = 0, tiles_y = 0, tiles_x = 0;
   int lds_floats = 0;
   int dbg_skip = 0;
@@ -54,6 +57,8 @@
   SegConvW pw1, pw2;
   SegDwW dw;
   long long skip_off = 0, lo2_off = 0, g_off = 0, lo_off = 0, part_lo_off = 0;
+  SegGate gate;
+  long long pre_gate_off = -1, cnt_off = -1;
   int TR = 0, TC = 0, tiles_y = 0, tiles_x = 0;
   int lds_floats = 0;
   int lo_floats = 0;
@@ -82,12 +87,14 @@
 constexpr int kSegLoTileFloats = 12 * 16 * kSegLoStride;
 constexpr int kSegScratchFloats = 640;
 constexpr int kSegGateStageFloats = 512 + 2 * (32 * 32 + 32);
+constexpr int kSegGateEpilogueFloats = kSegScratchFloats + kSegGateStageFloats;
 #ifndef BSX_SEG_RTC
 inline int seg_row_width(int cols) { return (cols + 15) / 16 * 16; }
 inline int seg_head_lds_floats(const SegHead& d) {
   const int AR = 2 * d.TR + 1, AC = 2 * d.TC + 1, IR = 2 * AR + 1, IC = 2 * AC + 1;
   const int win = (IR * IC * 3 + 3) & ~3;
-  return (win > 512 ? win : 512) + AR * AC * 16;
+  const int v = (win > 512 ? win : 512) + AR * AC * 16;
+  return v > kSegGateEpilogueFloats ? v : kSegGateEpilogueFloats;
 }
 inline int seg_k2_lds_floats(const SegK2& d) { const int v = 2 * (2 * d.TR + 1) * seg_row_width(2 * d.TC + 1) * 16; return kSegScratchFloats + (v > kSegGateStageFloats ? v : kSegGateStageFloats); }
 inline void seg_up_axis(int o, float scale, bool half_pixel, int in_size, int* lo, int* hi) {
@@ -115,7 +122,10 @@
   const int need = (lr + 1) * (lc + 1) * kSegLoStride;
   return need < kSegLoTileFloats ? need : kSegLoTileFloats;
 }
-inline int seg_k3_lds_floats(const SegK3& d) { return kSegScratchFloats + (d.TR + 2) * 256 + (d.lo_floats > 0 ? d.lo_floats : kSegLoTileFloats); }
+inline int seg_k3_lds_floats(const SegK3& d) {
+  const int v = kSegScratchFloats + (d.TR + 2) * 256 + (d.lo_floats > 0 ? d.lo_floats : kSegLoTileFloats);
+  return v > kSegGateEpilogueFloats ? v : kSegGateEpilogueFloats;
+}
 inline int seg_tail_lds_floats(const SegTail& d) { const int v = (d.TR + 2) * 256; return kSegScratchFloats + (v > kSegGateStageFloats ? v : kSegGateStageFloats) + (d.lo_floats > 0 ? d.lo_floats : kSegLoTileFloats); }
 #endif
 
diff --git a/include/bsx.h b/include/bsx.h
--- a/include/bsx.h
+++ b/include/bsx.h
@@ -124,6 +124,8 @@
 
 BSX_API int bsx_debug_mask_tile_stats(bsx_ctx* ctx, int n, long* out4);
 
+BSX_API int bsx_debug_seg_gates(bsx_ctx* ctx, int n, float* out);
+
 BSX_API int bsx_debug_program_timeline(bsx_ctx* ctx, int n, unsigned long long* ticks, int cap, void* stream);
 
 BSX_API int bsx_debug_gauss_coeffs(int ksize, int shift, uint32_t* c4 , uint32_t* c2 );
```

After: 732,300 (median of 6 runs). Within noise of the previous version (+0.9%).
